# wustl-cig/FLAIR

Hardware: AMD Instinct MI355X
Metric: restored frames/sec at 256x256, 16-frame clip, 250-step DDIM (higher is better)
Workload: dtype bf16

## Files before the change

flair_amd/csrc/conv.hip:

```cpp
#include <type_traits>

#include "common.h"

namespace {

struct ConvArgs {
    const void* x[4];
    int segC[4];
    int segLd[4];
    int nseg;
    const void* w;
    const float* bias;
    const void* res0;
    const void* res1;
    int res0Ld, res1Ld;
    void* y;
    int yLd;
    int T, H, W;
    int KT, KH, KW;
    int Cout, CinTot;
    int act;
    float outScale;
    long P;
    int nPixTiles, nCoTiles;
    int tFast;
    unsigned segBytes[4];
    unsigned wBytes;
    float* part;
    int splitK;
    const float* fbias;
    int fbiasLd;
    int stride;
    int tapShift;
    int reflect;
    float actParam;
    int actPeriod;
    int Hin, Win;
    int esz;
};

template <typename E> struct Mma;

template <> struct Mma<bf16_t> {
    static constexpr int BKE = 32;
    static __device__ __forceinline__ int chunk(int i, int half) { return 2 * i + half; }
    static __device__ __forceinline__ void run(const uint4 (&a)[2], const uint4 (&b)[2], f32x16& acc) {
        acc = __builtin_amdgcn_mfma_f32_32x32x16_bf16(__builtin_bit_cast(bf16x8, a[0]),
                                                      __builtin_bit_cast(bf16x8, b[0]), acc, 0, 0, 0);
        acc = __builtin_amdgcn_mfma_f32_32x32x16_bf16(__builtin_bit_cast(bf16x8, a[1]),
                                                      __builtin_bit_cast(bf16x8, b[1]), acc, 0, 0, 0);
    }
    static __device__ __forceinline__ void run1(const uint4& a, const uint4& b, f32x16& acc) {
        acc = __builtin_amdgcn_mfma_f32_32x32x16_bf16(__builtin_bit_cast(bf16x8, a), __builtin_bit_cast(bf16x8, b),
                                                      acc, 0, 0, 0);
    }
    static constexpr int MFMA_PER_HALF = 1;
};

template <> struct Mma<float> {
    static constexpr int BKE = 16;
    static __device__ __forceinline__ int chunk(int i, int half) { return 2 * half + i; }
    static __device__ __forceinline__ void run(const uint4 (&a)[2], const uint4 (&b)[2], f32x16& acc) {
        const float* af = reinterpret_cast<const float*>(a);
        const float* bf = reinterpret_cast<const float*>(b);
#pragma unroll
        for (int s = 0; s < 8; ++s)
            acc = __builtin_amdgcn_mfma_f32_32x32x2f32(af[s], bf[s], acc, 0, 0, 0);
    }
    static __device__ __forceinline__ void run1(const uint4& a, const uint4& b, f32x16& acc) {
        const float* af = reinterpret_cast<const float*>(&a);
        const float* bf = reinterpret_cast<const float*>(&b);
#pragma unroll
        for (int s = 0; s < 4; ++s)
            acc = __builtin_amdgcn_mfma_f32_32x32x2f32(af[s], bf[s], acc, 0, 0, 0);
    }
    static constexpr int MFMA_PER_HALF = 4;
};

__device__ __forceinline__ int lds_off(int row, int chunk) {
    return row * 64 + ((chunk ^ ((row >> 2) & 3)) << 4);
}

__device__ __forceinline__ int staged_row(int id) {
    const int g = id >> 3;
    return (g >> 2) * 8 + (g & 3) + 4 * ((id >> 2) & 1);
}

template <typename E>
__device__ __forceinline__ void store_quad(const ConvArgs& a, long p, int co, float v0, float v1, float v2, float v3) {
    if (co >= a.Cout) return;
    float v[4] = {v0, v1, v2, v3};
    if (a.bias) {
        const float4 b = *reinterpret_cast<const float4*>(a.bias + co);
// ... 133 lines not shown
        }
    }
}

template <typename E, int TH, int RPW, int PF>
__global__ __launch_bounds__(64 * TH / RPW, (2 * 64 * TH / RPW + 255) / 256)
void conv3x3_halo_kernel(ConvArgs a) {
    prefetch_kernargs<sizeof(ConvArgs)>();
    constexpr int BKE = Mma<E>::BKE;
    constexpr int VEC = ET<E>::VEC;
    constexpr int NT = 64 * TH / RPW;
    constexpr int HW_ = 34;
    constexpr int PITCH = 80;
    constexpr int HALO_ROWS = (TH + 2) * HW_;
    constexpr int HALO_PIECES = (HALO_ROWS + 7) / 8 * 8 * 4;
    constexpr int W_PIECES = 64 * 9 * 4;
    constexpr int HI = (HALO_PIECES + NT - 1) / NT;
    constexpr int WI = (W_PIECES + NT - 1) / NT;
    constexpr int HALO_BYTES = (TH + 2) * HW_ * PITCH;
    extern __shared__ __attribute__((aligned(16))) char smem[];
    char* sh = smem;
    char* sw = smem + HALO_BYTES;

    const int tid = threadIdx.x, lane = tid & 63, wave = tid >> 6;
    const int lr = lane & 31, lh = lane >> 5;
    const int bid = xcd_remap(blockIdx.x, gridDim.x);
    const int coTile = bid % a.nCoTiles;
    int rest = bid / a.nCoTiles;
    const int tilesW = a.W / 32, tilesH = (a.H + TH - 1) / TH;
    const int tw = rest % tilesW;
    rest /= tilesW;
    const int th = rest % tilesH;
    const int t = rest / tilesH;
    const int h0 = th * TH, w0 = tw * 32, co0 = coTile * 64;
    const int taps = a.KT * 9;
    const int pt = a.KT / 2;

    uint4 hreg[PF][HI], wreg[PF][WI];
    int dt = -pt, seg = 0, cb = 0, segOff = 0;
    auto dt_valid = [&](int d) { return (unsigned)(t + d) < (unsigned)a.T; };
    while (dt <= pt && !dt_valid(dt)) ++dt;

    constexpr unsigned ESZ = sizeof(E);
    int hpix[HI];
    unsigned hq[HI], woff[WI];
#pragma unroll
    for (int i = 0; i < HI; ++i) {
        const int id = i * NT + tid;
        const int pix = staged_row(id);
        const int r = pix / HW_, c = pix % HW_;
        const int hh = h0 + r - 1, ww = w0 + c - 1;
        const bool ok = pix < HALO_ROWS && (unsigned)hh < (unsigned)a.H && (unsigned)ww < (unsigned)a.W;
        hpix[i] = ok ? hh * a.W + ww : -1;
        hq[i] = (id & 3) * VEC * ESZ;
    }
    const __amdgpu_buffer_rsrc_t wrs = make_rsrc(a.w, a.wBytes);
#pragma unroll
    for (int i = 0; i < WI; ++i) {
        const int id = i * NT + tid;
        const int row = staged_row(id);
        const int co = row / 9, tap9 = row % 9;
        const bool ok = id < W_PIECES && co0 + co < a.Cout;
        woff[i] = ok ? (unsigned)(((co0 + co) * taps + tap9) * a.CinTot + (id & 3) * VEC) * ESZ : FLAIR_OOB;
    }

    auto issue = [&](uint4 (&hr)[HI], uint4 (&wr)[WI]) {
        const unsigned ld = (unsigned)a.segLd[seg] * ESZ;
        const char* frame = reinterpret_cast<const char*>(a.x[seg]) + (size_t)(t + dt) * a.H * a.W * ld;
        const __amdgpu_buffer_rsrc_t xr = make_rsrc(frame, a.segBytes[seg]);
        const unsigned cofs = (unsigned)(cb * BKE) * ESZ;
#pragma unroll
        for (int i = 0; i < HI; ++i) {
            const unsigned off = hpix[i] >= 0 ? (unsigned)hpix[i] * ld + cofs + hq[i] : FLAIR_OOB;
            hr[i] = buf_load16(xr, off);
        }
        const unsigned kofs = (unsigned)((dt + pt) * 9 * a.CinTot + segOff + cb * BKE) * ESZ;
#pragma unroll
        for (int i = 0; i < WI; ++i) wr[i] = buf_load16(wrs, woff[i] == FLAIR_OOB ? FLAIR_OOB : woff[i] + kofs);
    };
    auto advance = [&]() {
        ++cb;
        if (cb * BKE >= a.segC[seg]) {
            cb = 0;
            segOff += a.segC[seg];
            if (++seg >= a.nseg) {
                seg = 0;
                segOff = 0;
                ++dt;
                while (dt <= pt && !dt_valid(dt)) ++dt;
            }
        }
    };
    auto write_lds = [&](const uint4 (&hr)[HI], const uint4 (&wr)[WI]) {
#pragma unroll
        for (int i = 0; i < HI; ++i) {
            const int id = i * NT + tid;
            const int row = staged_row(id);
            if (row < HALO_ROWS) *reinterpret_cast<uint4*>(sh + row * PITCH + (id & 3) * 16) = hr[i];
        }
#pragma unroll
        for (int i = 0; i < WI; ++i) {
            const int id = i * NT + tid;
            if (id < W_PIECES) *reinterpret_cast<uint4*>(sw + staged_row(id) * PITCH + (id & 3) * 16) = wr[i];
        }
    };
    int nValidDt = 0;
    for (int d = -pt; d <= pt; ++d) nValidDt += dt_valid(d) ? 1 : 0;
    const int nch = nValidDt * (a.CinTot / BKE);

    f32x16 acc[RPW][2];
#pragma unroll
    for (int j = 0; j < RPW; ++j)
#pragma unroll
        for (int i = 0; i < 2; ++i)
#pragma unroll
            for (int r = 0; r < 16; ++r) acc[j][i][r] = 0.f;

    auto compute = [&]() {
        const char* hb = sh + ((wave * RPW * HW_) + lr) * PITCH;
        const char* wb0 = sw + (lr * 9) * PITCH;
        const char* wb1 = sw + ((lr + 32) * 9) * PITCH;
        uint4 fa0[2][2], fa1[2][2], fb[2][RPW][2];
        auto load_tap = [&](int set, int tap9) {
            const int kh = tap9 / 3, kw = tap9 % 3;
            fa0[set][0] = *reinterpret_cast<const uint4*>(wb0 + tap9 * PITCH + 16 * Mma<E>::chunk(0, lh));
            fa0[set][1] = *reinterpret_cast<const uint4*>(wb0 + tap9 * PITCH + 16 * Mma<E>::chunk(1, lh));
            fa1[set][0] = *reinterpret_cast<const uint4*>(wb1 + tap9 * PITCH + 16 * Mma<E>::chunk(0, lh));
            fa1[set][1] = *reinterpret_cast<const uint4*>(wb1 + tap9 * PITCH + 16 * Mma<E>::chunk(1, lh));
#pragma unroll
            for (int j = 0; j < RPW; ++j) {
                const char* hp = hb + ((j + kh) * HW_ + kw) * PITCH;
                fb[set][j][0] = *reinterpret_cast<const uint4*>(hp + 16 * Mma<E>::chunk(0, lh));
                fb[set][j][1] = *reinterpret_cast<const uint4*>(hp + 16 * Mma<E>::chunk(1, lh));
            }
        };
        load_tap(0, 0);
        __builtin_amdgcn_sched_group_barrier(0x100, 4 + 2 * RPW, 0);
#pragma unroll
        for (int tap9 = 0; tap9 < 9; ++tap9) {
            const int set = tap9 & 1;
            if (tap9 < 8) load_tap(set ^ 1, tap9 + 1);
#pragma unroll
            for (int j = 0; j < RPW; ++j) {
                Mma<E>::run(fa0[set], fb[set][j], acc[j][0]);
                Mma<E>::run(fa1[set], fb[set][j], acc[j][1]);
            }
            if (tap9 < 8) __builtin_amdgcn_sched_group_barrier(0x100, 4 + 2 * RPW, 0);
            __builtin_amdgcn_sched_group_barrier(0x8, (sizeof(E) == 2 ? 4 : 16) * RPW, 0);
        }
    };

    int issued = 0;
#pragma unroll
    for (int s_ = 0; s_ < PF; ++s_)
        if (issued < nch) {
            issue(hreg[s_], wreg[s_]);
            advance();
            ++issued;
        }
    write_lds(hreg[0], wreg[0]);
    __syncthreads();
    for (int k = 0; k < nch; k += PF) {
#pragma unroll
        for (int par = 0; par < PF; ++par) {
            const int kk = k + par;
            if (kk < nch) {
                if (issued < nch) {
                    issue(hreg[par], wreg[par]);
                    advance();
                    ++issued;
                }
                compute();
                if (kk + 1 < nch) {
                    __syncthreads();
                    write_lds(hreg[(par + 1) % PF], wreg[(par + 1) % PF]);
                    __syncthreads();
                }
            }
        }
    }

    if ((a.Cout & 7) == 0) {
        constexpr int VEC = ET<E>::VEC;
        constexpr int CHUNKS = 64 / VEC;
        __syncthreads();
#pragma unroll
        for (int j = 0; j < RPW; ++j) {
            char* tile = smem + (wave * RPW + j) * 32 * (64 * 4 + 16);
#pragma unroll
            for (int i = 0; i < 2; ++i)
#pragma unroll
// ... 84 lines not shown
}

template <typename E, int TH, int RPW, int CF>
__global__ __launch_bounds__(256 * TH / RPW / CF, (256 * TH / RPW / CF) / 256) void conv3x3_halo_ks_kernel(ConvArgs a) {
    static_assert(RPW == 1 && CF == 2, "one image row and both 32-cout fragments per wave");
    prefetch_kernargs<sizeof(ConvArgs)>();
    constexpr int NRG = TH / RPW;
    constexpr int NCG = 2 / CF;
    constexpr int NW = 2 * NRG * NCG, NT = 64 * NW;
    constexpr int BKE = Mma<E>::BKE;
    constexpr int VEC = ET<E>::VEC;
    constexpr unsigned ESZ = sizeof(E);
    constexpr int HW_ = 34, PITCH = 80;
    constexpr int HALO_ROWS = (TH + 2) * HW_;
    constexpr int HALO_PIECES = (HALO_ROWS + 7) / 8 * 8 * 4;
    constexpr int W_PIECES = 64 * 9 * 4;
    constexpr int HI = (HALO_PIECES + NT - 1) / NT;
    constexpr int WI = (W_PIECES + NT - 1) / NT;
    constexpr int HALO_BYTES = (TH + 2) * HW_ * PITCH;
    constexpr int STAGE_BYTES = HALO_BYTES + 64 * 9 * PITCH;
    extern __shared__ __attribute__((aligned(16))) char smem[];

    const int tid = threadIdx.x, lane = tid & 63, wave = tid >> 6;
    const int lr = lane & 31, lh = lane >> 5;
    const int rp = wave % NRG, kh2 = (wave / NRG) & 1, cg = wave / (2 * NRG);
    const int bid = xcd_remap(blockIdx.x, gridDim.x);
    const int coTile = bid % a.nCoTiles;
    int rest = bid / a.nCoTiles;
    const int tilesW = a.W / 32, tilesH = (a.H + TH - 1) / TH;
    const int tw = rest % tilesW;
    rest /= tilesW;
    const int th = rest % tilesH;
    const int t = rest / tilesH;
    const int h0 = th * TH, w0 = tw * 32, co0 = coTile * 64;
    const int taps = a.KT * 9;
    const int pt = a.KT / 2;

    float biasv[VEC];
    {
        const int bco = co0 + (lane % (64 / VEC)) * VEC;
#pragma unroll
        for (int e = 0; e < VEC; ++e) biasv[e] = (a.bias && bco < a.Cout) ? a.bias[bco + e] : 0.f;
    }
    uint4 hreg[HI], wreg[WI];
    int dt = -pt, seg = 0, cb = 0, segOff = 0;
    auto dt_valid = [&](int d) { return (unsigned)(t + d) < (unsigned)a.T; };
    while (dt <= pt && !dt_valid(dt)) ++dt;

    int hpix[HI];
    unsigned hq[HI], woff[WI];
#pragma unroll
    for (int i = 0; i < HI; ++i) {
        const int id = i * NT + tid;
        const int pix = staged_row(id);
        const int r = pix / HW_, c = pix % HW_;
        const int hh = h0 + r - 1, ww = w0 + c - 1;
        const bool ok = pix < HALO_ROWS && (unsigned)hh < (unsigned)a.H && (unsigned)ww < (unsigned)a.W;
        hpix[i] = ok ? hh * a.W + ww : -1;
        hq[i] = (id & 3) * VEC * ESZ;
    }
    const __amdgpu_buffer_rsrc_t wrs = make_rsrc(a.w, a.wBytes);
#pragma unroll
    for (int i = 0; i < WI; ++i) {
        const int id = i * NT + tid;
        const int row = staged_row(id);
        const int co = row / 9, tap9 = row % 9;
        const bool ok = id < W_PIECES && co0 + co < a.Cout;
        woff[i] = ok ? (unsigned)(((co0 + co) * taps + tap9) * a.CinTot + (id & 3) * VEC) * ESZ : FLAIR_OOB;
    }
    auto issue = [&]() {
        const unsigned ld = (unsigned)a.segLd[seg] * ESZ;
        const char* frame = reinterpret_cast<const char*>(a.x[seg]) + (size_t)(t + dt) * a.H * a.W * ld;
        const __amdgpu_buffer_rsrc_t xr = make_rsrc(frame, a.segBytes[seg]);
        const unsigned cofs = (unsigned)(cb * BKE) * ESZ;
#pragma unroll
        for (int i = 0; i < HI; ++i)
            hreg[i] = buf_load16(xr, hpix[i] >= 0 ? (unsigned)hpix[i] * ld + cofs + hq[i] : FLAIR_OOB);
        const unsigned kofs = (unsigned)((dt + pt) * 9 * a.CinTot + segOff + cb * BKE) * ESZ;
#pragma unroll
        for (int i = 0; i < WI; ++i) wreg[i] = buf_load16(wrs, woff[i] == FLAIR_OOB ? FLAIR_OOB : woff[i] + kofs);
        ++cb;
        if (cb * BKE >= a.segC[seg]) {
            cb = 0;
            segOff += a.segC[seg];
            if (++seg >= a.nseg) {
                seg = 0;
                segOff = 0;
                ++dt;
                while (dt <= pt && !dt_valid(dt)) ++dt;
            }
        }
    };
    auto write_lds = [&](int stage) {
        char* sh = smem + stage * STAGE_BYTES;
        char* sw = sh + HALO_BYTES;
#pragma unroll
        for (int i = 0; i < HI; ++i) {
            const int id = i * NT + tid;
            const int row = staged_row(id);
            if (row < HALO_ROWS) *reinterpret_cast<uint4*>(sh + row * PITCH + (id & 3) * 16) = hreg[i];
        }
#pragma unroll
        for (int i = 0; i < WI; ++i) {
            const int id = i * NT + tid;
            if (id < W_PIECES) *reinterpret_cast<uint4*>(sw + staged_row(id) * PITCH + (id & 3) * 16) = wreg[i];
        }
    };
    int nValidDt = 0;
    for (int d = -pt; d <= pt; ++d) nValidDt += dt_valid(d) ? 1 : 0;
    const int nch = nValidDt * (a.CinTot / BKE);

    f32x16 acc[RPW][CF];
#pragma unroll
    for (int j = 0; j < RPW; ++j)
#pragma unroll
        for (int i = 0; i < CF; ++i)
#pragma unroll
            for (int r = 0; r < 16; ++r) acc[j][i][r] = 0.f;

    const int ck = 16 * Mma<E>::chunk(kh2, lh);
    auto compute = [&](int stage) {
        const char* sh = smem + stage * STAGE_BYTES;
        const char* hb = sh + ((RPW * rp * HW_) + lr) * PITCH + ck;
        const char* wb0 = sh + HALO_BYTES + ((cg * CF * 32 + lr) * 9) * PITCH + ck;
        uint4 fa[2][CF], fb[2][RPW];
        auto load_tap = [&](int set, int tap9) {
            const int kh = tap9 / 3, kw = tap9 % 3;
#pragma unroll
            for (int i = 0; i < CF; ++i)
                fa[set][i] = *reinterpret_cast<const uint4*>(wb0 + (i * 32 * 9 + tap9) * PITCH);
#pragma unroll
            for (int j = 0; j < RPW; ++j)
                fb[set][j] = *reinterpret_cast<const uint4*>(hb + ((kh + j) * HW_ + kw) * PITCH);
        };
        load_tap(0, 0);
        __builtin_amdgcn_sched_group_barrier(0x100, CF + RPW, 0);
#pragma unroll
        for (int tap9 = 0; tap9 < 9; ++tap9) {
            const int set = tap9 & 1;
            if (tap9 < 8) load_tap(set ^ 1, tap9 + 1);
#pragma unroll
            for (int j = 0; j < RPW; ++j)
#pragma unroll
                for (int i = 0; i < CF; ++i) Mma<E>::run1(fa[set][i], fb[set][j], acc[j][i]);
            if (tap9 < 8) __builtin_amdgcn_sched_group_barrier(0x100, CF + RPW, 0);
            __builtin_amdgcn_sched_group_barrier(0x8, CF * RPW * Mma<E>::MFMA_PER_HALF, 0);
        }
    };

    issue();
    write_lds(0);
    if (nch > 1) issue();
    __syncthreads();
    for (int k = 0; k < nch; ++k) {
        compute(k & 1);
        if (k + 1 < nch) {
            write_lds((k + 1) & 1);
            if (k + 2 < nch) issue();
            __syncthreads();
        }
    }

    constexpr int FPITCH = 64 * 4 + 16;
    constexpr int CHUNKS = 64 / VEC;
    constexpr int PARTS = NW / TH;
    constexpr int NIT = 32 * CHUNKS / 64 / PARTS;
    const int orow = wave % TH, part = wave / TH;
    const int h = h0 + orow;
    const long prow = ((long)t * a.H + h) * a.W + w0;
    const int ech = lane % CHUNKS;
    const int eco = co0 + ech * VEC;
    const bool eok = h < a.H && eco < a.Cout;
    uint4 r0v[NIT], r1v[NIT];
#pragma unroll
    for (int k = 0; k < NIT; ++k) {
        const int px = ((k * PARTS + part) * 64 + lane) / CHUNKS;
        const long p = prow + px;
        r0v[k] = r1v[k] = make_uint4(0u, 0u, 0u, 0u);
        if (eok && a.res0) r0v[k] = *reinterpret_cast<const uint4*>(reinterpret_cast<const E*>(a.res0) + p * a.res0Ld + eco);
        if (eok && a.res1) r1v[k] = *reinterpret_cast<const uint4*>(reinterpret_cast<const E*>(a.res1) + p * a.res1Ld + eco);
    }
    __syncthreads();
#pragma unroll
    for (int pass = 0; pass < 2; ++pass) {
        if (kh2 == pass) {
#pragma unroll
            for (int j = 0; j < RPW; ++j) {
                char* tile = smem + (RPW * rp + j) * 32 * FPITCH + lr * FPITCH;
#pragma unroll
                for (int i = 0; i < CF; ++i)
#pragma unroll
                    for (int g = 0; g < 4; ++g) {
                        float4* dst = reinterpret_cast<float4*>(tile + ((cg * CF + i) * 32 + 8 * g + 4 * lh) * 4);
// ... 20 lines not shown
        float v[VEC];
        const float* src = reinterpret_cast<const float*>(tile + px * FPITCH) + ech * VEC;
#pragma unroll
        for (int e = 0; e < VEC; e += 4) {
            const float4 q = *reinterpret_cast<const float4*>(src + e);
            v[e] = q.x; v[e + 1] = q.y; v[e + 2] = q.z; v[e + 3] = q.w;
        }
#pragma unroll
        for (int e = 0; e < VEC; ++e) v[e] += biasv[e];
        if (a.fbias) {
            const float* fb = a.fbias + (long)t * a.fbiasLd + eco;
#pragma unroll
            for (int e = 0; e < VEC; ++e) v[e] += fb[e];
        }
        if (leaky) {
#pragma unroll
            for (int e = 0; e < VEC; ++e) v[e] = fmaxf(v[e], v[e] * slope);
        } else if (a.act == FLAIR_ACT_DCN_OFFSETS) {
            dcn_offset_act<VEC>(v, eco, a.actParam, a.actPeriod);
        } else if (a.act == FLAIR_ACT_SILU) {
#pragma unroll
            for (int e = 0; e < VEC; ++e) v[e] = silu_f(v[e]);
        } else {
#pragma unroll
            for (int e = 0; e < VEC; ++e) v[e] = apply_act(v[e], a.act);
        }
        if (a.res0) {
            float r[VEC];
            Vec16<E>::load(reinterpret_cast<const E*>(&r0v[k]), r);
#pragma unroll
            for (int e = 0; e < VEC; ++e) v[e] += r[e];
        }
        if (a.res1) {
            float r[VEC];
            Vec16<E>::load(reinterpret_cast<const E*>(&r1v[k]), r);
#pragma unroll
            for (int e = 0; e < VEC; ++e) v[e] += r[e];
        }
#pragma unroll
        for (int e = 0; e < VEC; ++e) v[e] *= a.outScale;
        Vec16<E>::store(reinterpret_cast<E*>(a.y) + p * a.yLd + eco, v);
    }
}

template <typename E, int TH, int RPW, int CF>
int launch_halo_ks(const ConvArgs& a0, hipStream_t s) {
    ConvArgs a = a0;
    a.nCoTiles = cdiv(a.Cout, 64);
    const int grid = a.T * cdiv(a.H, TH) * (a.W / 32) * a.nCoTiles;
    const size_t lds = 2 * ((size_t)(TH + 2) * 34 * 80 + 64 * 9 * 80);
    static LdsAttrOnce attr;
    {
        const hipError_t e = flair_max_lds_once(attr, reinterpret_cast<const void*>(&conv3x3_halo_ks_kernel<E, TH, RPW, CF>));
        FLAIR_CHECK(e == hipSuccess, "flair_conv_nhwc: hipFuncSetAttribute: %s", hipGetErrorString(e));
    }
    hipLaunchKernelGGL((conv3x3_halo_ks_kernel<E, TH, RPW, CF>), dim3(grid), dim3(256 * TH / RPW / CF), lds, s, a);
    FLAIR_LAUNCH_CHECK();
    return FLAIR_OK;
}

struct DmaTile {
    int t, h0, w0, co0;
};

template <int NW, int RPW, int NSTAGE>
__device__ __forceinline__ void conv3x3_dma_body(const ConvArgs& a, int nTiles, int tilesPerXcd) {
    using E = bf16_t;
    static_assert((RPW == 1 || RPW == 2) && NSTAGE == 2, "the clip-level and one-tile forms (two stages)");
    constexpr int KSTEPS = 2;
    constexpr int TH = NW * RPW, HWP = 34;
    constexpr int HALO_ROWS = (TH + 2) * HWP;
    constexpr int HALO_INSTR = (HALO_ROWS + 15) / 16;
    constexpr int W_INSTR = 64 * 9 / 16;
    constexpr int HALO_BYTES = HALO_INSTR * 1024;
    constexpr int STAGE_BYTES = HALO_BYTES + W_INSTR * 1024;
    constexpr int NSLOT = (HALO_INSTR + W_INSTR + NW - 1) / NW;
    constexpr int BIAS_OFF = NSTAGE * STAGE_BYTES + NW * 1024;
    extern __shared__ __attribute__((aligned(16))) char smem[];

    const int tid = threadIdx.x, lane = tid & 63;
    const int wave = __builtin_amdgcn_readfirstlane(tid >> 6);
    const int lr = lane & 31, lh = lane >> 5;
    const int taps = a.KT * 9, pt = a.KT / 2;
    const int chunksPerTap = a.CinTot / 32;
    const int H = a.H, W = a.W, T = a.T;

    const int xcd = blockIdx.x & 7, slot = blockIdx.x >> 3, slotsPerXcd = gridDim.x >> 3;
    const int tilesW = W / 32, tilesH = H / TH, nCoTiles = a.nCoTiles;
    auto tile_at = [&](int i, DmaTile& tl) -> bool {
        const int inXcd = slot + i * slotsPerXcd;
        const int id = xcd * tilesPerXcd + inXcd;
        if (inXcd >= tilesPerXcd || id >= nTiles) return false;
        int rest = id;
        tl.co0 = (rest % nCoTiles) * 64;
        rest /= nCoTiles;
        if (a.tFast) {
            tl.t = rest % T;
            rest /= T;
            tl.w0 = (rest % tilesW) * 32;
            tl.h0 = (rest / tilesW) * TH;
            return true;
        }
        tl.w0 = (rest % tilesW) * 32;
        rest /= tilesW;
        tl.h0 = (rest % tilesH) * TH;
        tl.t = rest / tilesH;
        return true;
    };

    const int lrow = lane >> 2, lchunk = lane & 3;
    unsigned slotv[NSLOT], hchunk[NSLOT];
#pragma unroll
    for (int i = 0; i < NSLOT; ++i) {
        const int id = wave * NSLOT + i;
        const int c = (id * 16 + lrow) % HWP;
        hchunk[i] = (unsigned)((lchunk ^ ((c >> 2) & 3)) << 4);
    }
    auto setup_tile = [&](const DmaTile& tl) {
#pragma unroll
        for (int i = 0; i < NSLOT; ++i) {
            const int id = wave * NSLOT + i;
            const int R = id * 16 + lrow;
            const int hr = R / HWP, c = R - hr * HWP;
            const int hh = tl.h0 - 1 + hr, ww = tl.w0 - 1 + c;
            const bool okh = R < HALO_ROWS && (unsigned)hh < (unsigned)H && (unsigned)ww < (unsigned)W;
            const unsigned hv = okh ? (unsigned)(hh * W + ww) : 0xffffffffu;
            const int row = R - HALO_INSTR * 16;
            const int tap9 = row >> 6, co = row & 63;
            const bool okw = row >= 0 && row < 576 && tl.co0 + co < a.Cout;
            const unsigned wv = okw ? (unsigned)(((tl.co0 + co) * taps + tap9) * a.CinTot) * 2u + ((lchunk ^ ((co >> 2) & 3)) << 4) : FLAIR_OOB;
            slotv[i] = id >= HALO_INSTR ? wv : hv;
        }
    };

    const u32x4_t wdesc = make_desc(a.w, a.wBytes);
    struct Walk {
        int dt, seg, cb, segOff, j;
    };
    auto dt_at = [&](int t, int j) { return a.tFast ? (j + a.KT * T - t) % a.KT - pt : j - pt; };
    auto walk_first = [&](int t, Walk& wk) {
        wk.j = 0; wk.seg = 0; wk.cb = 0; wk.segOff = 0;
        while (wk.j < a.KT && (unsigned)(t + dt_at(t, wk.j)) >= (unsigned)T) ++wk.j;
        wk.dt = dt_at(t, wk.j);
    };
    auto walk_next = [&](int t, Walk& wk) {
        ++wk.cb;
        if (wk.cb * 32 >= a.segC[wk.seg]) {
            wk.cb = 0;
            wk.segOff += a.segC[wk.seg];
            if (++wk.seg >= a.nseg) {
                wk.seg = 0;
                wk.segOff = 0;
                ++wk.j;
                while (wk.j < a.KT && (unsigned)(t + dt_at(t, wk.j)) >= (unsigned)T) ++wk.j;
                wk.dt = dt_at(t, wk.j);
            }
        }
    };
    auto chunks_of = [&](int t) {
        int n = 0;
        for (int d = -pt; d <= pt; ++d) n += (unsigned)(t + d) < (unsigned)T ? 1 : 0;
        return n * chunksPerTap;
    };
    auto issue = [&](const DmaTile& tl, const Walk& wk, int stage) {
        const unsigned ld = (unsigned)a.segLd[wk.seg] * 2u;
        const char* frame = reinterpret_cast<const char*>(a.x[wk.seg]) + (size_t)(tl.t + wk.dt) * H * W * ld;
        const u32x4_t xdesc = make_desc(frame, a.segBytes[wk.seg]);
        const unsigned cofs = (unsigned)(wk.cb * 64);
        const unsigned kofs = (unsigned)((wk.dt + pt) * 9 * a.CinTot + wk.segOff + wk.cb * 32) * 2u;
        const unsigned sbase = (unsigned)(stage * STAGE_BYTES + wave * NSLOT * 1024);
#pragma unroll
        for (int i = 0; i < NSLOT; ++i) {
            const bool isw = wave * NSLOT + i >= HALO_INSTR;
            const unsigned sv = slotv[i];
            const unsigned offh = sv == 0xffffffffu ? FLAIR_OOB : sv * ld + cofs + hchunk[i];
            const unsigned offw = sv == FLAIR_OOB ? FLAIR_OOB : sv + kofs;
            u32x4_t d;
            d.x = isw ? wdesc.x : xdesc.x;
            d.y = isw ? wdesc.y : xdesc.y;
            d.z = isw ? wdesc.z : xdesc.z;
            d.w = 0x00020000u;
            const bool idle = wave * NSLOT + i >= HALO_INSTR + W_INSTR;
            dma16(d, isw ? offw : offh, idle ? (unsigned)(NSTAGE * STAGE_BYTES + ((wave * NSLOT + i - HALO_INSTR - W_INSTR) % NW) * 1024) : sbase + i * 1024);
        }
    };

    unsigned aoff[KSTEPS], boff[3][KSTEPS];
#pragma unroll
    for (int s_ = 0; s_ < KSTEPS; ++s_) {
        aoff[s_] = (unsigned)(HALO_BYTES + lr * 64 + (((2 * s_ + lh) ^ ((lr >> 2) & 3)) << 4));
#pragma unroll
        for (int kw = 0; kw < 3; ++kw)
            boff[kw][s_] = (unsigned)((RPW * wave * HWP + kw + lr) * 64 + (((2 * s_ + lh) ^ (((kw + lr) >> 2) & 3)) << 4));
    }

    f32x16 acc[RPW][2];
    auto zero_acc = [&]() {
#pragma unroll
        for (int j = 0; j < RPW; ++j)
#pragma unroll
            for (int i = 0; i < 2; ++i)
#pragma unroll
                for (int r = 0; r < 16; ++r) acc[j][i][r] = 0.f;
    };
    auto compute = [&](int stage) {
        const char* sb = smem + stage * STAGE_BYTES;
        uint4 fb[2][RPW + 2][KSTEPS];
        uint4 fa[2][2][KSTEPS];
        auto load_b = [&](int set, int kw) {
#pragma unroll
            for (int h = 0; h < RPW + 2; ++h)
#pragma unroll
                for (int s_ = 0; s_ < KSTEPS; ++s_)
                    fb[set][h][s_] = *reinterpret_cast<const uint4*>(sb + h * (HWP * 64) + boff[kw][s_]);
        };
        auto load_a = [&](int set, int kh, int kw) {
#pragma unroll
            for (int cf = 0; cf < 2; ++cf)
#pragma unroll
                for (int s_ = 0; s_ < KSTEPS; ++s_)
                    fa[set][cf][s_] = *reinterpret_cast<const uint4*>(sb + (kh * 3 + kw) * 4096 + cf * 2048 + aoff[s_]);
        };
        load_b(0, 0);
        load_a(0, 0, 0);
        __builtin_amdgcn_sched_group_barrier(0x100, KSTEPS * (RPW + 2) + 2 * KSTEPS, 0);
#pragma unroll
        for (int step = 0; step < 9; ++step) {
            const int kq = step / 3, kh = step % 3;
            const int nkq = (step + 1) / 3, nkh = (step + 1) % 3;
            if (step < 8) {
                if (nkh == 0) load_b(nkq & 1, nkq);
                load_a((step + 1) & 1, nkh, nkq);
            }
#pragma unroll
            for (int j = 0; j < RPW; ++j)
#pragma unroll
                for (int cf = 0; cf < 2; ++cf) Mma<E>::run(fa[step & 1][cf], fb[kq & 1][j + kh], acc[j][cf]);
            if (step < 8) {
                if (nkh == 0) __builtin_amdgcn_sched_group_barrier(0x100, KSTEPS * (RPW + 2) + 2 * KSTEPS, 0);
// ... 209 lines not shown
            if (more) {
                walk_first(nxt.t, wk);
                setup_tile(nxt);
                remIssue = chunks_of(nxt.t);
                bias_request(nxt);
            }
        }
        if (more) {
            issue(nxt, wk, stage ^ 1);
            walk_next(nxt.t, wk);
            --remIssue;
        }
        compute(stage);
        if (biasPending) bias_commit(iNxt);
        bool storesInFlight = false;
        if (--remCompute == 0) {
            epilogue(cur, iCur);
            storesInFlight = RPW >= 2 ? !a.res1 : cur.co0 + 64 <= a.Cout && !res0any;
            ++iCur;
            if (!tile_at(iCur, cur)) break;
            remCompute = chunks_of(cur.t);
            zero_acc();
        }
        if (storesInFlight) {
            asm volatile("s_waitcnt vmcnt(%0)" ::"n"(4 * RPW) : "memory");
        } else {
            asm volatile("s_waitcnt vmcnt(0)" ::: "memory");
        }
        __syncthreads();
        stage ^= 1;
    }
}

template <int NW, int RPW, int NSTAGE>
__global__ __launch_bounds__(64 * NW, (NW + 3) / 4) void conv3x3_dma_kernel(ConvArgs a, int nTiles, int tilesPerXcd) {
    prefetch_kernargs<sizeof(ConvArgs) + 8>();
    conv3x3_dma_body<NW, RPW, NSTAGE>(a, nTiles, tilesPerXcd);
}

template <int NW, int RPW, int NSTAGE>
int launch_dma(const ConvArgs& a0, hipStream_t s) {
    constexpr int TH = NW * RPW;
    ConvArgs a = a0;
    a.nCoTiles = cdiv(a.Cout, 64);
    a.tFast = a.KT == 3 && a.T > 1;
    const int nTiles = a.T * (a.H / TH) * (a.W / 32) * a.nCoTiles;
    const int nCu = flair_cu_count();
    int grid = nTiles < nCu ? (nTiles + 7) / 8 * 8 : nCu / 8 * 8;
    if (grid < 8) grid = 8;
    const int tilesPerXcd = (nTiles + 7) / 8;
    constexpr int HALO_INSTR = ((TH + 2) * 34 + 15) / 16;
    const size_t lds = NSTAGE * (size_t)(HALO_INSTR + 36) * 1024 + NW * 1024 + 512;
    static LdsAttrOnce attr;
    {
        const hipError_t e = flair_max_lds_once(attr, reinterpret_cast<const void*>(&conv3x3_dma_kernel<NW, RPW, NSTAGE>));
        FLAIR_CHECK(e == hipSuccess, "flair_conv_nhwc: hipFuncSetAttribute: %s", hipGetErrorString(e));
    }
    hipLaunchKernelGGL((conv3x3_dma_kernel<NW, RPW, NSTAGE>), dim3(grid), dim3(64 * NW), lds, s, a, nTiles, tilesPerXcd);

    FLAIR_LAUNCH_CHECK();
    return FLAIR_OK;
}


template <bool HALO3>
__global__ __launch_bounds__(512, 2) void conv_frame_kernel(ConvArgs a) {
    static_assert(HALO3, "halo ring of three, weight ring of two");
    prefetch_kernargs<sizeof(ConvArgs)>();
    using E = bf16_t;
    constexpr int NW = 8, HWP = 34;
    constexpr int HINSTR = 22, HIMG = HINSTR * 1024, WINSTR = 36, SLOT = WINSTR * 1024;
    constexpr int HR = 3, WR = 2;
    constexpr int RING = HR * HIMG, BIAS = RING + WR * SLOT;
    constexpr int NH = (HINSTR + NW - 1) / NW, NWS = (WINSTR + NW - 1) / NW;
    extern __shared__ __attribute__((aligned(16))) char smem[];
    const int tid = threadIdx.x, lane = tid & 63;
    const int wave = __builtin_amdgcn_readfirstlane(tid >> 6);
    const int lr = lane & 31, lh = lane >> 5;
    const int lrow = lane >> 2, lchunk = lane & 3;
    const int tilesW = a.W / 32, perFrame = tilesW * (a.H / 8);
    const int bid = xcd_remap(blockIdx.x, gridDim.x);
    const int t = bid / perFrame, tile = bid - t * perFrame;
    const int h0 = (tile / tilesW) * 8, w0 = (tile % tilesW) * 32;
    const int nS = a.CinTot / 32;

    const u32x4_t wdesc = make_desc(a.w, a.wBytes);
    const u32x4_t bdesc = make_desc(a.bias, a.bias ? (unsigned)a.Cout * 4u : 0u);
    dma16(bdesc, (unsigned)(lane * 16), (unsigned)BIAS);
    unsigned hpix[NH], hpiece[NH];
#pragma unroll
    for (int i = 0; i < NH; ++i) {
        const int k = (wave * NH + i) % HINSTR;
        const int R = k * 16 + lrow;
        const int hr = R / HWP, c = R - hr * HWP;
        const int hh = h0 - 1 + hr, ww = w0 - 1 + c;
        const bool ok = R < 10 * HWP && (unsigned)hh < (unsigned)a.H && (unsigned)ww < (unsigned)a.W;
        hpix[i] = ok ? (unsigned)(hh * a.W + ww) : 0xffffffffu;
        hpiece[i] = (unsigned)((lchunk ^ ((c >> 2) & 3)) << 4);
    }
    unsigned wlane[NWS];
#pragma unroll
    for (int i = 0; i < NWS; ++i) {
        const int id = (wave * NWS + i) % WINSTR;
        const int row = id * 16 + lrow, tap9 = row >> 6, co = row & 63;
        wlane[i] = co < a.Cout ? (unsigned)((co * 9 + tap9) * a.CinTot) * 2u + (unsigned)((lchunk ^ ((co >> 2) & 3)) << 4) : FLAIR_OOB;
    }
    int hseg = 0, hcb = 0;
    auto issue_halo = [&](int slot) {
        const unsigned ld = (unsigned)a.segLd[hseg] * 2u;
        const u32x4_t xdesc = make_desc(reinterpret_cast<const char*>(a.x[hseg]) + (size_t)t * a.H * a.W * ld, a.segBytes[hseg]);
        const unsigned cofs = (unsigned)(hcb * 64);
#pragma unroll
        for (int i = 0; i < NH; ++i) {
            const int k = (wave * NH + i) % HINSTR;
            dma16(xdesc, hpix[i] == 0xffffffffu ? FLAIR_OOB : hpix[i] * ld + cofs + hpiece[i], (unsigned)(slot * HIMG + k * 1024));
        }
        if (++hcb * 32 >= a.segC[hseg]) {
            hcb = 0;
            ++hseg;
        }
    };
    auto issue_w = [&](int s_) {
#pragma unroll
        for (int i = 0; i < NWS; ++i) {
            const int id = (wave * NWS + i) % WINSTR;
            dma16(wdesc, wlane[i] == FLAIR_OOB ? FLAIR_OOB : wlane[i] + (unsigned)(s_ * 64), (unsigned)(RING + (s_ % WR) * SLOT + id * 1024));
        }
    };
    issue_halo(0);
    issue_w(0);
    if (nS > 1) {
        issue_halo(1);
        issue_w(1);
    }
    if (nS > 2) issue_halo(2);

    unsigned aoff[2], boff[3][2];
#pragma unroll
    for (int ks = 0; ks < 2; ++ks) {
        aoff[ks] = (unsigned)(lr * 64 + (((2 * ks + lh) ^ ((lr >> 2) & 3)) << 4));
#pragma unroll
        for (int kw = 0; kw < 3; ++kw)
            boff[kw][ks] = (unsigned)((wave * HWP + kw + lr) * 64 + (((2 * ks + lh) ^ (((kw + lr) >> 2) & 3)) << 4));
    }
    f32x16 acc[2];
    auto compute = [&](int wslot, int hslot) {
        const char* wb = smem + RING + wslot * SLOT;
        const char* xb = smem + hslot * HIMG;
        uint4 fb[2][3][2], fa[2][2][2];
        auto load_b = [&](int set, int kw) {
#pragma unroll
            for (int h = 0; h < 3; ++h)
#pragma unroll
                for (int ks = 0; ks < 2; ++ks) fb[set][h][ks] = *reinterpret_cast<const uint4*>(xb + h * (HWP * 64) + boff[kw][ks]);
        };
        auto load_a = [&](int set, int kh, int kw) {
#pragma unroll
            for (int cf = 0; cf < 2; ++cf)
#pragma unroll
                for (int ks = 0; ks < 2; ++ks) fa[set][cf][ks] = *reinterpret_cast<const uint4*>(wb + (kh * 3 + kw) * 4096 + cf * 2048 + aoff[ks]);
        };
        load_b(0, 0);
        load_a(0, 0, 0);
#pragma unroll
        for (int step = 0; step < 9; ++step) {
            const int kq = step / 3, kh = step % 3;
            const int nkq = (step + 1) / 3, nkh = (step + 1) % 3;
            if (step < 8) {
                if (nkh == 0) load_b(nkq & 1, nkq);
                load_a((step + 1) & 1, nkh, nkq);
            }
#pragma unroll
            for (int cf = 0; cf < 2; ++cf)
#pragma unroll
                for (int ks = 0; ks < 2; ++ks)
                    acc[cf] = __builtin_amdgcn_mfma_f32_32x32x16_bf16(__builtin_bit_cast(bf16x8, fa[step & 1][cf][ks]), __builtin_bit_cast(bf16x8, fb[kq & 1][kh][ks]), acc[cf], 0, 0, 0);
        }
    };

    const long prow = ((long)t * a.H + h0 + wave) * a.W + w0;
    const unsigned yLdB = (unsigned)a.yLd * 2u, r0LdB = (unsigned)a.res0Ld * 2u, r1LdB = (unsigned)a.res1Ld * 2u;
    const __amdgpu_buffer_rsrc_t yd = make_rsrc(reinterpret_cast<char*>(a.y) + prow * a.yLd * 2, (unsigned)a.W * yLdB);
    const __amdgpu_buffer_rsrc_t r0d = make_rsrc(a.res0 ? reinterpret_cast<const char*>(a.res0) + prow * a.res0Ld * 2 : nullptr, a.res0 ? (unsigned)a.W * r0LdB : 0u);
    const __amdgpu_buffer_rsrc_t r1d = make_rsrc(a.res1 ? reinterpret_cast<const char*>(a.res1) + prow * a.res1Ld * 2 : nullptr, a.res1 ? (unsigned)a.W * r1LdB : 0u);
    uint4 r0v[4], r1v[4];
#pragma unroll
    for (int g = 0; g < 4; ++g) r0v[g] = r1v[g] = make_uint4(0u, 0u, 0u, 0u);

    for (int s_ = 0; s_ < nS; ++s_) {
        if (s_ + 1 >= nS) asm volatile("s_waitcnt vmcnt(0)" ::: "memory");
        else if (s_ == 0 && nS > 2) asm volatile("s_waitcnt vmcnt(%0)" ::"n"(2 * NH + NWS) : "memory");
        else if (s_ == 0) asm volatile("s_waitcnt vmcnt(%0)" ::"n"(NH + NWS) : "memory");
        else asm volatile("s_waitcnt vmcnt(%0)" ::"n"(NH) : "memory");
        __builtin_amdgcn_s_barrier();
        if (s_ == 0) {
            const float* sb = reinterpret_cast<const float*>(smem + BIAS);
#pragma unroll
            for (int cf = 0; cf < 2; ++cf)
#pragma unroll
                for (int g = 0; g < 4; ++g) {
                    const float4 bq = *reinterpret_cast<const float4*>(sb + cf * 32 + 8 * g + 4 * lh);
                    acc[cf][4 * g] = bq.x; acc[cf][4 * g + 1] = bq.y; acc[cf][4 * g + 2] = bq.z; acc[cf][4 * g + 3] = bq.w;
                }
        }
        if (s_ >= 1 && s_ + 1 < nS) issue_w(s_ + 1);
        if (s_ >= 1 && s_ + 2 < nS) issue_halo((s_ + 2) % 3);
        if (s_ + 1 == nS) {
            if (a.res0) {
#pragma unroll
// ... 27 lines not shown
            Vec16<E>::load(reinterpret_cast<const E*>(&r0v[g]), r);
#pragma unroll
            for (int e = 0; e < 8; ++e) v[e] += r[e];
            Vec16<E>::load(reinterpret_cast<const E*>(&r1v[g]), r);
#pragma unroll
            for (int e = 0; e < 8; ++e) v[e] = (v[e] + r[e]) * scale;
            alignas(16) E out[8];
            Vec16<E>::store(out, v);
            const uint4 ov = *reinterpret_cast<const uint4*>(out);
            const unsigned yo = 16 * g + 8 * lh < a.Cout ? (unsigned)lr * yLdB + (unsigned)(32 * g + 16 * lh) : FLAIR_OOB;
            __builtin_amdgcn_raw_buffer_store_b128(u32x4_t{ov.x, ov.y, ov.z, ov.w}, yd, (int)yo, 0, 0);
        }
}

static bool frame_kernel_ok(const ConvArgs& a) {
    if (a.esz != 2 || a.KT != 1 || a.KH != 3 || a.KW != 3 || a.stride != 1 || a.fbias || a.Cout > 64 || a.Cout % 8 || a.W % 32 || a.H % 8) return false;
    if (!(a.act == FLAIR_ACT_NONE || a.act == FLAIR_ACT_RELU || a.act == FLAIR_ACT_LRELU01 || a.act == FLAIR_ACT_LRELU02)) return false;
    if (a.tapShift || a.reflect || a.CinTot % 32 || a.CinTot < 32) return false;
    for (int i = 0; i < a.nseg; ++i)
        if (a.segC[i] % 32) return false;
    return true;
}

static int launch_frame(const ConvArgs& a, hipStream_t s) {
    constexpr size_t lds = (3 * 22 + 2 * 36) * 1024 + 1024;
    static LdsAttrOnce attr;
    const hipError_t e = flair_max_lds_once(attr, reinterpret_cast<const void*>(&conv_frame_kernel<true>));
    FLAIR_CHECK(e == hipSuccess, "flair_conv_nhwc: hipFuncSetAttribute: %s", hipGetErrorString(e));
    hipLaunchKernelGGL(conv_frame_kernel<true>, dim3(a.T * (a.H / 8) * (a.W / 32)), dim3(512), lds, s, a);
    FLAIR_LAUNCH_CHECK();
    return FLAIR_OK;
}

template <typename E, int TC, int TP, int WC, int WP, int PD, int KWID>
__global__ __launch_bounds__(256) void conv_igemm_kernel(ConvArgs a) {
    prefetch_kernargs<sizeof(ConvArgs)>();
    constexpr int BKE = Mma<E>::BKE * KWID;
    constexpr int ROWB = 64 * KWID;
    constexpr int CPR = 4 * KWID;
    constexpr int RPP = 256 / CPR;
    constexpr int VEC = ET<E>::VEC;
    constexpr int FC = TC / WC / 32;
    constexpr int FP = TP / WP / 32;
    constexpr int XR = TP / RPP;
    constexpr int WR = TC / RPP;
    static_assert(WC * WP == 4 && FC >= 1 && FP >= 1 && XR >= 1 && WR >= 1, "tile");

    extern __shared__ __attribute__((aligned(16))) char smem[];
    constexpr int BUF = (TC + TP) * ROWB;
    auto loff = [](int row, int chunk) { return KWID == 1 ? lds_off(row, chunk) : row * 128 + ((chunk ^ ((row >> 1) & 7)) << 4); };

    const int tid = threadIdx.x;
    const int lane = tid & 63, wave = __builtin_amdgcn_readfirstlane(tid >> 6);
    const int wc = wave / WP, wp = wave % WP;

    const int bid = xcd_remap(blockIdx.x, gridDim.x);
    const int coTile = bid % a.nCoTiles;
    const int pixTile = bid / a.nCoTiles;
    const long p0 = (long)pixTile * TP;
    const int co0 = coTile * TC;

    const int chunk = tid % CPR;
    const int srow = tid / CPR;
    int xt[XR], xh[XR], xw[XR];
    bool xvalid[XR];
#pragma unroll
    for (int i = 0; i < XR; ++i) {
        long p = p0 + srow + RPP * i;
        xvalid[i] = p < a.P;
        if (!xvalid[i]) p = 0;
        int w_ = (int)(p % a.W);
        long q = p / a.W;
        xw[i] = w_;
        xh[i] = (int)(q % a.H);
        xt[i] = (int)(q / a.H);
    }
    const int taps = a.KT * a.KH * a.KW;
    const int pt = a.KT / 2, ph = a.KH / 2, pw = a.KW / 2;
    const int tFirst = (int)(p0 / ((long)a.H * a.W));
    const int tileFrames = (int)((TP + (long)a.H * a.W - 1) / ((long)a.H * a.W)) + 1;

    uint4 xreg[PD][XR], wreg[PD][WR];

    const int nkAll = taps * (a.CinTot / BKE);
    const int ks0 = (int)((long)blockIdx.y * nkAll / a.splitK);
    const int ks1 = (int)((long)(blockIdx.y + 1) * nkAll / a.splitK);
    int tap = ks0 / (a.CinTot / BKE), seg = 0, cb = ks0 % (a.CinTot / BKE), segOff = 0;
    while (cb * BKE >= a.segC[seg]) {
        cb -= a.segC[seg] / BKE;
        segOff += a.segC[seg];
        ++seg;
    }
    int dw = tap % a.KW - pw, dh = (tap / a.KW) % a.KH - ph, dt = tap / (a.KW * a.KH) - pt;

    const __amdgpu_buffer_rsrc_t wrs = make_rsrc(a.w, a.wBytes);
    constexpr unsigned ESZ = sizeof(E);
    auto issue_loads = [&](int set) {
        const int ld = a.segLd[seg];
        int fb = tFirst + dt;
        fb = fb < 0 ? 0 : (fb >= a.T ? a.T - 1 : fb);
        int nfr = a.T - fb;
        if (nfr > tileFrames) nfr = tileFrames;
        const size_t frameBytes = (size_t)a.Hin * a.Win * ld * ESZ;
        const __amdgpu_buffer_rsrc_t xr =
            make_rsrc(reinterpret_cast<const char*>(a.x[seg]) + fb * frameBytes, (unsigned)(nfr * frameBytes));
        const int coff = cb * BKE + chunk * VEC;
#pragma unroll
        for (int i = 0; i < XR; ++i) {
            const int t2 = xt[i] + dt;
            int h2 = xh[i] * a.stride + dh + a.tapShift, w2 = xw[i] * a.stride + dw + a.tapShift;
            if (a.reflect) {
                h2 = h2 < 0 ? -h2 : (h2 >= a.Hin ? 2 * a.Hin - 2 - h2 : h2);
                w2 = w2 < 0 ? -w2 : (w2 >= a.Win ? 2 * a.Win - 2 - w2 : w2);
            }
            const bool ok = xvalid[i] && (unsigned)t2 < (unsigned)a.T && (unsigned)h2 < (unsigned)a.Hin &&
                            (unsigned)w2 < (unsigned)a.Win;
            const unsigned off = ok ? (unsigned)((((t2 - fb) * a.Hin + h2) * a.Win + w2) * ld + coff) * ESZ : FLAIR_OOB;
            xreg[set][i] = buf_load16(xr, off);
        }
        const unsigned kofs = (unsigned)(tap * a.CinTot + segOff + coff) * ESZ;
#pragma unroll
        for (int j = 0; j < WR; ++j) {
            const int n = co0 + srow + RPP * j;
            wreg[set][j] = buf_load16(wrs, n < a.Cout ? (unsigned)(n * taps * a.CinTot) * ESZ + kofs : FLAIR_OOB);
        }
    };
    auto advance = [&]() {
        ++cb;
        if (cb * BKE >= a.segC[seg]) {
            cb = 0;
            segOff += a.segC[seg];
            ++seg;
            if (seg >= a.nseg) {
                seg = 0;
                segOff = 0;
                ++tap;
                ++dw;
                if (dw > pw) {
                    dw = -pw;
                    ++dh;
                    if (dh > ph) {
                        dh = -ph;
                        ++dt;
                    }
                }
            }
        }
    };
    auto write_lds = [&](int buf, int set) {
        char* base = smem + buf * BUF;
#pragma unroll
        for (int j = 0; j < WR; ++j)
            *reinterpret_cast<uint4*>(base + loff(srow + RPP * j, chunk)) = wreg[set][j];
#pragma unroll
        for (int i = 0; i < XR; ++i)
            *reinterpret_cast<uint4*>(base + TC * ROWB + loff(srow + RPP * i, chunk)) = xreg[set][i];
    };

    f32x16 acc[FC][FP];
#pragma unroll
    for (int i = 0; i < FC; ++i)
#pragma unroll
        for (int j = 0; j < FP; ++j)
#pragma unroll
            for (int r = 0; r < 16; ++r) acc[i][j][r] = 0.f;

    const int nk = ks1 - ks0;
    const int lr = lane & 31, lh = lane >> 5;

#pragma unroll
    for (int u = 0; u < PD; ++u)
        if (u < nk) {
            issue_loads(u);
            advance();
        }
    write_lds(0, 0);
    __syncthreads();

    for (int ks = 0; ks < nk; ks += PD) {
#pragma unroll
        for (int u = 0; u < PD; ++u) {
            const int k = ks + u;
            if (k >= nk) break;
            const int cur = k & 1;
            if (k + PD < nk) {
                issue_loads(u);
                advance();
            }
            const char* wb = smem + cur * BUF;
            const char* xb = wb + TC * ROWB;
#pragma unroll
            for (int sp = 0; sp < KWID; ++sp) {
                uint4 af[FC][2], bfr[FP][2];
#pragma unroll
                for (int i = 0; i < FC; ++i) {
                    const int row = wc * (TC / WC) + i * 32 + lr;
                    af[i][0] = *reinterpret_cast<const uint4*>(wb + loff(row, 4 * sp + Mma<E>::chunk(0, lh)));
                    af[i][1] = *reinterpret_cast<const uint4*>(wb + loff(row, 4 * sp + Mma<E>::chunk(1, lh)));
                }
#pragma unroll
                for (int j = 0; j < FP; ++j) {
                    const int row = wp * (TP / WP) + j * 32 + lr;
                    bfr[j][0] = *reinterpret_cast<const uint4*>(xb + loff(row, 4 * sp + Mma<E>::chunk(0, lh)));
                    bfr[j][1] = *reinterpret_cast<const uint4*>(xb + loff(row, 4 * sp + Mma<E>::chunk(1, lh)));
                }
#pragma unroll
                for (int i = 0; i < FC; ++i)
#pragma unroll
                    for (int j = 0; j < FP; ++j) Mma<E>::run(af[i], bfr[j], acc[i][j]);
            }
            if (k + 1 < nk) write_lds(cur ^ 1, (u + 1) % PD);
            __syncthreads();
        }
    }

    if (a.splitK > 1) {
#pragma unroll
        for (int j = 0; j < FP; ++j) {
            const long p = p0 + wp * (TP / WP) + j * 32 + lr;
            if (p >= a.P) continue;
#pragma unroll
            for (int i = 0; i < FC; ++i)
#pragma unroll
                for (int g = 0; g < 4; ++g) {
                    const int co = co0 + wc * (TC / WC) + i * 32 + 8 * g + 4 * lh;
                    if (co < a.Cout)
                        *reinterpret_cast<float4*>(a.part + ((long)blockIdx.y * a.P + p) * a.Cout + co) =
                            make_float4(acc[i][j][4 * g], acc[i][j][4 * g + 1], acc[i][j][4 * g + 2],
                                        acc[i][j][4 * g + 3]);
                }
        }
        return;
    }
    if ((a.Cout & 7) == 0 && ((uintptr_t)a.y & 15) == 0 && (a.yLd * (int)sizeof(E)) % 16 == 0 &&
        (!a.res0 || (((uintptr_t)a.res0 & 15) == 0 && (a.res0Ld * (int)sizeof(E)) % 16 == 0)) &&
        (!a.res1 || (((uintptr_t)a.res1 & 15) == 0 && (a.res1Ld * (int)sizeof(E)) % 16 == 0))) {
        auto run = [&](auto actTag) {
            igemm_epilogue<E, decltype(actTag)::value, FC, FP>(a, acc, p0 + wp * (TP / WP), co0 + wc * (TC / WC), lr, lh);
        };
        if (a.act == FLAIR_ACT_DCN_OFFSETS) run(std::integral_constant<int, 1>{});
        else if (a.act == FLAIR_ACT_SILU) run(std::integral_constant<int, 2>{});
        else if (a.act == FLAIR_ACT_GELU) run(std::integral_constant<int, 3>{});
        else run(std::integral_constant<int, 0>{});
        return;
    }
#pragma unroll
    for (int j = 0; j < FP; ++j) {
        const long p = p0 + wp * (TP / WP) + j * 32 + lr;
        if (p >= a.P) continue;
#pragma unroll
        for (int i = 0; i < FC; ++i)
#pragma unroll
            for (int g = 0; g < 4; ++g)
                store_quad<E>(a, p, co0 + wc * (TC / WC) + i * 32 + 8 * g + 4 * lh, acc[i][j][4 * g],
                              acc[i][j][4 * g + 1], acc[i][j][4 * g + 2], acc[i][j][4 * g + 3]);
    }
}

template <typename E>
__global__ void conv_splitk_reduce_kernel(ConvArgs a) {
    const unsigned cq = (unsigned)(a.Cout / 4);
    const unsigned quads = (unsigned)a.P * cq;
    const size_t slice = (size_t)a.P * a.Cout;
    for (unsigned i = blockIdx.x * blockDim.x + threadIdx.x; i < quads; i += gridDim.x * blockDim.x) {
        const unsigned p = i / cq;
        const int co = (int)(i - p * cq) * 4;
        const float* src = a.part + (size_t)p * a.Cout + co;
        float4 s = make_float4(0.f, 0.f, 0.f, 0.f);
        int k = 0;
        for (; k + 4 <= a.splitK; k += 4) {
            float4 v[4];
#pragma unroll
            for (int u = 0; u < 4; ++u) v[u] = *reinterpret_cast<const float4*>(src + (size_t)(k + u) * slice);
#pragma unroll
            for (int u = 0; u < 4; ++u) {
                s.x += v[u].x; s.y += v[u].y; s.z += v[u].z; s.w += v[u].w;
            }
        }
        for (; k < a.splitK; ++k) {
            const float4 v = *reinterpret_cast<const float4*>(src + (size_t)k * slice);
            s.x += v.x; s.y += v.y; s.z += v.z; s.w += v.w;
        }
        store_quad<E>(a, p, co, s.x, s.y, s.z, s.w);
    }
}

template <typename E, int TC, int TP, int WC, int WP, int PD, int KWID>
int launch_pd(const ConvArgs& a0, hipStream_t s) {
    ConvArgs a = a0;
    a.nPixTiles = cdiv(a.P, TP);
    a.nCoTiles = cdiv(a.Cout, TC);
    const int grid = a.nPixTiles * a.nCoTiles;
    const size_t lds = 2 * (TC + TP) * 64 * KWID;
    hipLaunchKernelGGL((conv_igemm_kernel<E, TC, TP, WC, WP, PD, KWID>), dim3(grid, a.splitK), dim3(256), lds, s, a);
    FLAIR_LAUNCH_CHECK();
    if (a.splitK > 1) {
        long g = (a.P * (a.Cout / 4) + 255) / 256;
        if (g > 2048) g = 2048;
        hipLaunchKernelGGL(conv_splitk_reduce_kernel<E>, dim3((int)g), dim3(256), 0, s, a);
        FLAIR_LAUNCH_CHECK();
    }
    return FLAIR_OK;
}

template <typename E, int TC, int TP, int WC, int WP>
int launch(const ConvArgs& a, hipStream_t s) {
    if constexpr (sizeof(E) == 2) {
        bool ok = true;
        for (int i = 0; i < a.nseg; ++i) ok = ok && a.segC[i] % 64 == 0;
        if (ok) return launch_pd<E, TC, TP, WC, WP, 2, 2>(a, s);
    }
    return launch_pd<E, TC, TP, WC, WP, 4, 1>(a, s);
}

int choose_split(const ConvArgs& a, int variant) {
    if (variant > 2) return 1;
    const int maxBlocks = variant == 0 ? 512 : 1024, maxSplit = 16;
    const int tc = variant == 0 ? 128 : 64, tp = variant == 2 ? 64 : 128;
    const int bke = 64 / (a.wBytes && a.CinTot ? (int)(a.wBytes / ((unsigned long long)a.Cout * a.KT * a.KH * a.KW * a.CinTot)) : 2);
    const long nk = (long)a.KT * a.KH * a.KW * (a.CinTot / bke);
    const long tiles = (long)cdiv(a.P, tp) * cdiv(a.Cout, tc);
    if (tiles >= 384 || nk < 32) return 1;
    long s = maxBlocks / tiles;
    if (s > maxSplit) s = maxSplit;
    if (s > nk / 8) s = nk / 8;
    return s < 1 ? 1 : (int)s;
}

int choose_variant(const ConvArgs& a) {
    if (!a.reflect && a.stride == 1 && a.KH == 3 && a.KW == 3 && a.W % 32 == 0 && a.H >= 2) {
        const long per = (long)a.T * (a.W / 32) * cdiv(a.Cout, 64);
        const bool ks = a.Cout % 8 == 0;
        if (a.esz == 2 && ks && a.act != FLAIR_ACT_GELU && a.H % 16 == 0 && per * cdiv(a.H, 8) > 256 && per * (a.H / 16) >= 192) return 8;
        const bool dmaOk = a.esz == 2 && ks && a.act != FLAIR_ACT_GELU;
        if (per * cdiv(a.H, 8) >= 256) return ks && per * cdiv(a.H, 8) <= 256 ? (dmaOk && a.H % 8 == 0 ? 9 : 6) : 3;
        if (per * cdiv(a.H, 4) >= 256) return ks && per * cdiv(a.H, 4) <= 256 ? 7 : 4;
        return 5;
    }
    const long tiles128 = (long)cdiv(a.P, 128) * cdiv(a.Cout, 128);
    if (a.Cout > 64 && tiles128 >= 512) return 0;
    if (a.Cout >= 128 && a.P >= 1024 && tiles128 <= 64 && (long)a.KT * a.KH * a.KW * a.CinTot >= 2304) return 0;
    const long tiles64x128 = (long)cdiv(a.P, 128) * cdiv(a.Cout, 64);
    if (tiles64x128 >= 512) return 1;
    return 2;
}

template <typename E>
int dispatch(const ConvArgs& a0, hipStream_t s) {
    ConvArgs a = a0;
    const int variant = choose_variant(a);
    a.splitK = a.part ? choose_split(a, variant) : 1;
    switch (variant) {
        case 0: return launch<E, 128, 128, 2, 2>(a, s);
        case 1: return launch<E, 64, 128, 1, 4>(a, s);
        case 2: return launch<E, 64, 64, 2, 2>(a, s);
        case 3: return launch_halo<E, 8, 1, 1>(a, s);
        case 4: return launch_halo<E, 4, 1, 1>(a, s);
        case 6: return launch_halo_ks<E, 8, 1, 2>(a, s);
        case 7: return launch_halo_ks<E, 4, 1, 2>(a, s);
        case 8: return launch_dma<8, 2, 2>(a, s);
        case 9:
            if (frame_kernel_ok(a)) return launch_frame(a, s);
            return launch_dma<8, 1, 2>(a, s);
        default: return launch_halo<E, 2, 1, 1>(a, s);
    }
}

}

extern "C" int flair_conv_variant(const flair_conv_params* p);

static void fill_geometry(ConvArgs& a, const flair_conv_params* p) {
    a.stride = p->stride > 1 ? p->stride : 1;
    a.Hin = p->H; a.Win = p->W;
    a.T = p->T; a.KT = p->KT; a.KH = p->KH; a.KW = p->KW; a.Cout = p->Cout;
    a.reflect = p->reflect_pad ? 1 : 0;
    a.act = p->act;
    a.H = (p->H + a.stride - 1) / a.stride;
    a.W = (p->W + a.stride - 1) / a.stride;
    a.P = (long)p->T * a.H * a.W;
    a.CinTot = 0;
    for (int i = 0; i < p->nseg && i < 4; ++i) a.CinTot += p->seg_c[i];
    const int esz = p->dtype == FLAIR_BF16 ? 2 : 4;
    a.esz = esz;
    a.wBytes = (unsigned)((unsigned long long)p->Cout * p->KT * p->KH * p->KW * a.CinTot * esz);
}

extern "C" size_t flair_conv_workspace_bytes(const flair_conv_params* p) {
    if (!p) return 0;
    ConvArgs a{};
    fill_geometry(a, p);
    const int split = choose_split(a, choose_variant(a));
    return split > 1 ? (size_t)split * a.P * a.Cout * sizeof(float) : 0;
}

extern "C" int flair_conv_nhwc(const flair_conv_params* p, const void* const* x, const void* w,
                               const float* bias, const float* frame_bias, const void* res0, const void* res1,
                               void* y, void* workspace, size_t workspace_bytes, hipStream_t stream) {
    FLAIR_CHECK(p && x && w && y, "flair_conv_nhwc: null argument");
    FLAIR_CHECK(p->dtype == FLAIR_F32 || p->dtype == FLAIR_BF16, "flair_conv_nhwc: bad dtype %d", p->dtype);
    FLAIR_CHECK(p->nseg >= 1 && p->nseg <= 4, "flair_conv_nhwc: nseg %d not in 1..4", p->nseg);
    FLAIR_CHECK(p->T > 0 && p->H > 0 && p->W > 0 && p->Cout > 0, "flair_conv_nhwc: empty shape");
    FLAIR_CHECK((p->KT & 1) && (p->KH & 1) && (p->KW & 1), "flair_conv_nhwc: kernel taps must be odd");
    FLAIR_CHECK(p->Cout % 4 == 0, "flair_conv_nhwc: Cout %d must be a multiple of 4", p->Cout);
    const int bke = p->dtype == FLAIR_BF16 ? 32 : 16;
    const int esz = p->dtype == FLAIR_BF16 ? 2 : 4;
    ConvArgs a{};
    a.CinTot = 0;
    for (int i = 0; i < p->nseg; ++i) {
        FLAIR_CHECK(x[i], "flair_conv_nhwc: segment %d is null", i);
        FLAIR_CHECK(p->seg_c[i] > 0 && p->seg_c[i] % bke == 0,
                    "flair_conv_nhwc: segment %d has %d channels; must be a multiple of %d", i, p->seg_c[i], bke);
        FLAIR_CHECK(p->seg_ld[i] >= p->seg_c[i] && (p->seg_ld[i] * esz) % 16 == 0 &&
                        ((uintptr_t)x[i]) % 16 == 0,
                    "flair_conv_nhwc: segment %d stride/alignment", i);
        a.x[i] = x[i];
        a.segC[i] = p->seg_c[i];
        a.segLd[i] = p->seg_ld[i];
        a.CinTot += p->seg_c[i];
        const unsigned long long bytes = (unsigned long long)p->H * p->W * p->seg_ld[i] * esz;
        FLAIR_CHECK(bytes < 0x40000000ull, "flair_conv_nhwc: one frame of segment %d spans %llu bytes (limit 1 GiB)",
                    i, bytes);
        a.segBytes[i] = (unsigned)bytes;
    }
    {
        const unsigned long long wb = (unsigned long long)p->Cout * p->KT * p->KH * p->KW * a.CinTot * esz;
        FLAIR_CHECK(wb < 0x80000000ull, "flair_conv_nhwc: weights span %llu bytes (limit 2 GiB)", wb);
        a.wBytes = (unsigned)wb;
    }
    const int gran = (p->dtype == FLAIR_BF16 && p->Cout % 8 != 0) ? 8 : 16;
    FLAIR_CHECK(p->y_ld >= p->Cout && (p->y_ld * esz) % gran == 0 && ((uintptr_t)y) % 16 == 0,
                "flair_conv_nhwc: output stride/alignment (y_ld = %d: >= Cout = %d, a multiple of %d bytes; y 16-byte aligned)",
                p->y_ld, p->Cout, gran);
    FLAIR_CHECK(!res0 || (p->res_ld[0] >= p->Cout && (p->res_ld[0] * esz) % gran == 0 && ((uintptr_t)res0) % gran == 0),
                "flair_conv_nhwc: res0 stride/alignment (res_ld = %d: >= Cout = %d; stride and pointer multiples of %d bytes)",
                p->res_ld[0], p->Cout, gran);
    FLAIR_CHECK(!res1 || (p->res_ld[1] >= p->Cout && (p->res_ld[1] * esz) % gran == 0 && ((uintptr_t)res1) % gran == 0),
                "flair_conv_nhwc: res1 stride/alignment (res_ld = %d: >= Cout = %d; stride and pointer multiples of %d bytes)",
                p->res_ld[1], p->Cout, gran);
    FLAIR_CHECK(((uintptr_t)w) % 16 == 0, "flair_conv_nhwc: weight alignment");
    FLAIR_CHECK(!bias || ((uintptr_t)bias) % 16 == 0, "flair_conv_nhwc: bias alignment");
    a.nseg = p->nseg;
    a.w = w;
    a.bias = bias;
    a.fbias = frame_bias;
    a.fbiasLd = p->frame_bias_ld;
    FLAIR_CHECK(!frame_bias || p->frame_bias_ld >= p->Cout, "flair_conv_nhwc: frame_bias_ld");
    {
        const unsigned long long hw = (unsigned long long)p->H * p->W * esz;
        FLAIR_CHECK(hw * p->y_ld < 0x40000000ull && (!res0 || hw * p->res_ld[0] < 0x40000000ull) && (!res1 || hw * p->res_ld[1] < 0x40000000ull),
                    "flair_conv_nhwc: one frame of the output / a residual spans more than 1 GiB");
    }
    a.res0 = res0;
    a.res1 = res1;
    a.res0Ld = p->res_ld[0];
    a.res1Ld = p->res_ld[1];
    a.y = y;
    a.yLd = p->y_ld;
    a.act = p->act;
    a.actParam = p->act_param;
    a.actPeriod = p->act_period;
    FLAIR_CHECK(p->act != FLAIR_ACT_DCN_OFFSETS || (p->act_period > 0 && p->act_period % 24 == 0),
                "flair_conv_nhwc: FLAIR_ACT_DCN_OFFSETS needs act_period = 3 * deform_groups (multiple of 24), got %d",
                p->act_period);
    a.outScale = p->out_scale;
    {
        ConvArgs g{};
        fill_geometry(g, p);
        a.stride = g.stride; a.Hin = g.Hin; a.Win = g.Win; a.T = g.T; a.H = g.H; a.W = g.W; a.P = g.P;
        a.KT = g.KT; a.KH = g.KH; a.KW = g.KW; a.Cout = g.Cout; a.esz = g.esz;
    }
    FLAIR_CHECK(a.stride == 1 || a.stride == 2, "flair_conv_nhwc: stride %d unsupported", p->stride);
    FLAIR_CHECK(!p->asym_pad || (a.stride == 2 && a.KH == a.KW && a.KT == 1 && p->H % 2 == 0 && p->W % 2 == 0),
                "flair_conv_nhwc: asym_pad needs a square 2-D stride-2 kernel on even frames");
    a.tapShift = p->asym_pad ? a.KH / 2 : 0;
    FLAIR_CHECK(!p->reflect_pad || (!p->asym_pad && a.KT == 1 && p->H > a.KH / 2 && p->W > a.KW / 2),
                "flair_conv_nhwc: reflect_pad needs a 2-D kernel smaller than the frame");
    a.reflect = p->reflect_pad ? 1 : 0;
    a.part = nullptr;
    a.splitK = 1;

    if (workspace && workspace_bytes >= flair_conv_workspace_bytes(p) && flair_conv_workspace_bytes(p) > 0) {
        FLAIR_CHECK(((uintptr_t)workspace) % 16 == 0, "flair_conv_nhwc: workspace alignment");
        a.part = reinterpret_cast<float*>(workspace);
    }
    if (p->dtype == FLAIR_BF16) return dispatch<bf16_t>(a, stream);
    return dispatch<float>(a, stream);
}

extern "C" int flair_conv_variant(const flair_conv_params* p) {
    if (!p) return -1;
    ConvArgs a{};
    fill_geometry(a, p);
    return choose_variant(a);
}
```

flair_amd/csrc/dcn.hip:

```cpp


#include "common.h"

namespace {

struct DcnArgs {
    const void* x[2];
    int xLd[2];
    int Cin;
    const void* raw; int rawLd;
    const float* flow1;
    const float* flow2;
    const void* w;
    const float* bias;
    void* y; int yLd;
    int F, H, W, Cout, G;
    float maxMag;
    int activated;
    long P;
    unsigned xBytes[2], rawBytes, wBytes;
};

template <typename E> struct MmaD;
template <> struct MmaD<bf16_t> {
// ... 29 lines not shown

__device__ __forceinline__ unsigned cvt_pk_bf16(float lo, float hi) {
    unsigned r;
    asm("v_cvt_pk_bf16_f32 %0, %1, %2" : "=v"(r) : "v"(lo), "v"(hi));
    return r;
}

__device__ __forceinline__ float fast_tanh(float x) {
    const float e = __expf(2.f * x);
    return 1.f - 2.f * __builtin_amdgcn_rcpf(e + 1.f);
}

template <typename E, int NCF, int NPF, int TPP, int OFFS, bool ONEFRAME, int PFD, bool DOT2>
__global__ __launch_bounds__(32 * NPF * TPP, (PFD == 1 ? 8 : NCF >= 4 ? 32 * NPF * TPP / 256 : 4)) void dcn_kernel(DcnArgs a) {
    static_assert(DOT2 == (sizeof(E) == 2 && OFFS == 1 && ONEFRAME), "the dot2 blend exactly for the bf16 per-frame activated forms");
    static_assert(OFFS != 2 || !ONEFRAME, "raw offsets: the general (batched) form only");
    prefetch_kernargs<sizeof(DcnArgs)>();
    constexpr int NT = 32 * NPF * TPP, NW = NT / 64;

    constexpr int TP = 32 * NPF, TC = 32 * NCF, CPR = TPP;
    constexpr int VEC = ET<E>::VEC;
    constexpr unsigned ESZ = sizeof(E);
    constexpr int BKE = CPR * VEC;
    constexpr int NPAIR = NCF * NPF;
    constexpr int KSPLIT = NW > NPAIR ? NW / NPAIR : 1;
    constexpr int PAIRS = NW > NPAIR ? 1 : NPAIR / NW;
    constexpr int KSUB = CPR / 4 / KSPLIT;
    static_assert((NW > NPAIR ? NPAIR * KSPLIT == NW : PAIRS * NW == NPAIR) && KSUB >= 1 && KSUB * KSPLIT * 4 == CPR,
                  "tile shape");
    constexpr int WR = (TC * CPR + NT - 1) / NT;
    constexpr int RAWR = (TP * 3 * (int)ESZ + NT - 1) / NT;
    constexpr int BUF = (TC + TP) * CPR * 16;
    extern __shared__ __attribute__((aligned(16))) char smem[];
    const int G = a.G;
    const int slabBytes = OFFS == 2 ? (3 * G * (int)ESZ + 15) & ~15 : 3 * G * (int)ESZ;
    const int slabPieces = slabBytes / 16;
    const int rawPitch = slabBytes + 16;
    char* sraw = smem;
    char* stile = smem + 2 * TP * rawPitch;

    const int tid = threadIdx.x, lane = tid & 63, wave = tid >> 6;
    const int lr = lane & 31, lh = lane >> 5;
    const long p0 = (long)xcd_remap(blockIdx.x, gridDim.x) * TP;
    const int q = tid % TPP, srow = tid / TPP;
    long p = p0 + srow;
    const bool pvalid = p < a.P;
    if (!pvalid) p = a.P - 1;
    const int pw = (int)(p % a.W);
    const int ph = (int)((p / a.W) % a.H);
    const int pf = (int)((ONEFRAME ? p0 : p) / ((long)a.W * a.H));
    float2 fl1 = make_float2(0.f, 0.f), fl2 = make_float2(0.f, 0.f);
    if (a.flow1) fl1 = *reinterpret_cast<const float2*>(a.flow1 + p * 2);
    if (a.flow2) fl2 = *reinterpret_cast<const float2*>(a.flow2 + p * 2);

    const __amdgpu_buffer_rsrc_t rr = make_rsrc(a.raw, a.rawBytes);
    auto raw_issue = [&](int tap, uint4 (&reg)[RAWR]) {
#pragma unroll
        for (int j = 0; j < RAWR; ++j) {
            const int id = tid + j * NT;
            const int px = id / slabPieces, pc = id - px * slabPieces;
            const long pp = p0 + px;
            const unsigned within = (unsigned)(3 * tap * G) * ESZ + pc * 16;
            reg[j] = buf_load16(rr, px < TP && pp < a.P ? (unsigned)(pp * a.rawLd * ESZ) + within : FLAIR_OOB);
        }
    };
    auto raw_write = [&](int tap, const uint4 (&reg)[RAWR]) {
#pragma unroll
        for (int j = 0; j < RAWR; ++j) {
            const int id = tid + j * NT;
            const int px = id / slabPieces, pc = id - px * slabPieces;
            if (px < TP) *reinterpret_cast<uint4*>(sraw + ((tap & 1) * TP + px) * rawPitch + pc * 16) = reg[j];
        }
    };
    auto stage_raw = [&](int tap) {
        uint4 reg[RAWR];
        raw_issue(tap, reg);
        raw_write(tap, reg);
    };

    const int cpg = a.Cin / G;
    int cpgShift = 0;
    while ((1 << cpgShift) < cpg) ++cpgShift;
    const int halfC = a.Cin / 2;
    const int cbPerTap = a.Cin / BKE;
    const int nk = 9 * cbPerTap;
    const size_t fo0 = ONEFRAME ? (size_t)pf * a.H * a.W * a.xLd[0] * ESZ : 0, fo1 = ONEFRAME ? (size_t)pf * a.H * a.W * a.xLd[1] * ESZ : 0;
    const __amdgpu_buffer_rsrc_t xr0 = make_rsrc(reinterpret_cast<const char*>(a.x[0]) + fo0, a.xBytes[0]);
    const __amdgpu_buffer_rsrc_t xr1 = make_rsrc(reinterpret_cast<const char*>(a.x[1]) + fo1, a.xBytes[1]);
    const __amdgpu_buffer_rsrc_t wrs = make_rsrc(a.w, a.wBytes);
    const unsigned frameBase = (unsigned)pf * a.H * a.W;

    struct Regs {
        uint4 c[4];
        uint4 w[WR];
        float wt[4];
    } rs[PFD];

    unsigned wrow[WR];
#pragma unroll
    for (int j = 0; j < WR; ++j) {
        const int id = tid + j * NT;
        const int n = id / CPR, ch = id % CPR;
        wrow[j] = n < a.Cout && n < TC ? (unsigned)(n * 9 * a.Cin + ch * VEC) * ESZ : FLAIR_OOB;
    }
    int itap = 0, icb = 0, ikh = 0, ikw = 0;
    const int rawRow = srow * rawPitch;
    const float fH = (float)a.H, fW = (float)a.W;
    const float phm1 = (float)(ph - 1), pwm1 = (float)(pw - 1);
    auto issue = [&](Regs& r) {
        const int tap = itap, cb = icb;
        const int c = cb * BKE + q * VEC;
        const int g = c >> cpgShift;
        const E* myraw = reinterpret_cast<const E*>(sraw + (tap & 1) * TP * rawPitch + rawRow);
        const float ry = ET<E>::ld(myraw + 2 * g), rx = ET<E>::ld(myraw + 2 * g + 1);
        const float rm = ET<E>::ld(myraw + 2 * G + g);
        const bool second = cb * BKE >= halfC;
        const float2 fl = second ? fl2 : fl1;
        float sy = phm1 + (float)ikh + fl.y, sx = pwm1 + (float)ikw + fl.x, mk;
        if constexpr (OFFS == 1) {
            sy += ry;
            sx += rx;
            mk = rm;
        } else if constexpr (OFFS == 2) {
            sy += ry;
            sx += rx;
            mk = __builtin_amdgcn_rcpf(1.f + __expf(-rm));
        } else {
            sy += a.maxMag * fast_tanh(ry);
            sx += a.maxMag * fast_tanh(rx);
            mk = __builtin_amdgcn_rcpf(1.f + __expf(-rm));
        }
        const float fy = floorf(sy), fx = floorf(sx);
        const float ay = sy - fy, ax = sx - fx;
        const int y0 = (int)__builtin_amdgcn_fmed3f(fy, -2.f, fH), x0 = (int)__builtin_amdgcn_fmed3f(fx, -2.f, fW);
        const unsigned ld = (unsigned)(second ? a.xLd[1] : a.xLd[0]) * ESZ;
        const unsigned coff = (unsigned)(c - (second ? halfC : 0)) * ESZ;
        const __amdgpu_buffer_rsrc_t xr = second ? xr1 : xr0;
        const unsigned rowStep = (unsigned)a.W * ld;
        if constexpr (ONEFRAME) {
            const float wx0 = (unsigned)x0 < (unsigned)a.W ? (1.f - ax) * mk : 0.f;
            const float wx1 = (unsigned)(x0 + 1) < (unsigned)a.W ? ax * mk : 0.f;
            r.wt[0] = (1.f - ay) * wx0;
            r.wt[1] = (1.f - ay) * wx1;
            r.wt[2] = ay * wx0;
            r.wt[3] = ay * wx1;
            const unsigned o00 =
                (unsigned)mul_i24(mul_i24(y0, a.W) + x0, (int)ld) + coff;
            r.c[0] = buf_load16(xr, o00);
            r.c[1] = buf_load16(xr, o00 + ld);
            r.c[2] = buf_load16(xr, o00 + rowStep);
            r.c[3] = buf_load16(xr, o00 + rowStep + ld);
        } else {
            r.wt[0] = (1.f - ay) * (1.f - ax) * mk;
            r.wt[1] = (1.f - ay) * ax * mk;
            r.wt[2] = ay * (1.f - ax) * mk;
            r.wt[3] = ay * ax * mk;
            const unsigned o00 = (unsigned)mul_i24(
                                     (int)frameBase + mul_i24(y0, a.W) + x0, (int)ld) + coff;
            const bool yok0 = pvalid && (unsigned)y0 < (unsigned)a.H, yok1 = pvalid && (unsigned)(y0 + 1) < (unsigned)a.H;
            const bool xok0 = (unsigned)x0 < (unsigned)a.W, xok1 = (unsigned)(x0 + 1) < (unsigned)a.W;
            r.c[0] = buf_load16(xr, yok0 && xok0 ? o00 : FLAIR_OOB);
            r.c[1] = buf_load16(xr, yok0 && xok1 ? o00 + ld : FLAIR_OOB);
            r.c[2] = buf_load16(xr, yok1 && xok0 ? o00 + rowStep : FLAIR_OOB);
            r.c[3] = buf_load16(xr, yok1 && xok1 ? o00 + rowStep + ld : FLAIR_OOB);
        }
        const unsigned wk = (unsigned)(tap * a.Cin + cb * BKE) * ESZ;
#pragma unroll
// ... 35 lines not shown
            outv = make_uint4(o[0], o[1], o[2], o[3]);
        } else if constexpr (sizeof(E) == 2) {
            typedef float f32x2 __attribute__((ext_vector_type(2)));
            f32x2 lo[2] = {{0.f, 0.f}, {0.f, 0.f}}, hi[2] = {{0.f, 0.f}, {0.f, 0.f}};
#pragma unroll
            for (int i = 0; i < 4; ++i) {
                const unsigned d[4] = {r.c[i].x, r.c[i].y, r.c[i].z, r.c[i].w};
                const f32x2 w = {r.wt[i], r.wt[i]};
#pragma unroll
                for (int j = 0; j < 2; ++j) {
                    const f32x2 vl = {__uint_as_float(d[2 * j] << 16), __uint_as_float(d[2 * j + 1] << 16)};
                    const f32x2 vh = {__uint_as_float(d[2 * j] & 0xffff0000u), __uint_as_float(d[2 * j + 1] & 0xffff0000u)};
                    lo[j] = __builtin_elementwise_fma(w, vl, lo[j]);
                    hi[j] = __builtin_elementwise_fma(w, vh, hi[j]);
                }
            }
            outv = make_uint4(cvt_pk_bf16(lo[0].x, hi[0].x), cvt_pk_bf16(lo[0].y, hi[0].y), cvt_pk_bf16(lo[1].x, hi[1].x),
                              cvt_pk_bf16(lo[1].y, hi[1].y));
        } else {
            float acc[VEC];
#pragma unroll
            for (int e = 0; e < VEC; ++e) acc[e] = 0.f;
#pragma unroll
            for (int i = 0; i < 4; ++i) {
                float v[VEC];
                Vec16<E>::load(reinterpret_cast<const E*>(&r.c[i]), v);
#pragma unroll
                for (int e = 0; e < VEC; ++e) acc[e] = fmaf(r.wt[i], v[e], acc[e]);
            }
            alignas(16) E out[VEC];
            Vec16<E>::store(out, acc);
            outv = *reinterpret_cast<const uint4*>(out);
        }
        *reinterpret_cast<uint4*>(base + TC * CPR * 16 + tile_off<CPR>(srow, q)) = outv;
#pragma unroll
        for (int j = 0; j < WR; ++j) {
            const int id = tid + j * NT;
            if (id < TC * CPR) *reinterpret_cast<uint4*>(base + tile_off<CPR>(id / CPR, id % CPR)) = r.w[j];
        }
    };

    f32x16 acc[PAIRS];
#pragma unroll
    for (int i = 0; i < PAIRS; ++i)
#pragma unroll
        for (int r = 0; r < 16; ++r) acc[i][r] = 0.f;

    constexpr int LEAD = PFD + 1;
    int stageTap = 0;
    {
        uint4 r0[RAWR], r1[RAWR];
        const bool two = cbPerTap - LEAD < 0;
        raw_issue(0, r0);
        if (two) raw_issue(1, r1);
        raw_write(0, r0);
        if (two) raw_write(1, r1);
        stageTap = two ? 2 : 1;
    }
    int stageAt = stageTap * cbPerTap - LEAD;
    __syncthreads();
    auto mfma_step = [&](int buf) {
        const char* wb = stile + buf * BUF;
        const char* xb = wb + TC * CPR * 16;
#pragma unroll
        for (int i = 0; i < PAIRS; ++i) {
            const int pair = KSPLIT > 1 ? wave % NPAIR : wave * PAIRS + i;
            const int kpart = KSPLIT > 1 ? wave / NPAIR : 0;
            const int pfrag = pair % NPF, cf = pair / NPF;
#pragma unroll
            for (int kk = 0; kk < KSUB; ++kk) {
                const int ks = kpart * KSUB + kk;
                uint4 af[2], bf[2];
#pragma unroll
                for (int h = 0; h < 2; ++h) {
                    const int ch = ks * 4 + MmaD<E>::chunk(h, lh);
                    bf[h] = *reinterpret_cast<const uint4*>(xb + tile_off<CPR>(pfrag * 32 + lr, ch));
                    af[h] = *reinterpret_cast<const uint4*>(wb + tile_off<CPR>(cf * 32 + lr, ch));
                }
                MmaD<E>::run(af, bf, acc[i]);
            }
        }
    };
#pragma unroll
    for (int u = 0; u < PFD - 1; ++u)
        if (u < nk) issue(rs[u]);
    constexpr int UNR = 2 * PFD;
    for (int k = 0; k < nk; k += UNR) {
#pragma unroll
        for (int u = 0; u < UNR; ++u) {
            if (k + u < nk) {
                if (k + u + PFD - 1 < nk) issue(rs[(u + PFD - 1) % PFD]);
                blend_and_stage(rs[u % PFD], u & 1);
                __syncthreads();
                mfma_step(u & 1);
                if (k + u == stageAt && stageTap < 9) {
                    stage_raw(stageTap);
                    ++stageTap;
                    stageAt += cbPerTap;
                }
            }
        }
    }
    if constexpr (KSPLIT > 1) {
        __syncthreads();
        float* red = reinterpret_cast<float*>(stile);
        const int pair0 = wave % NPAIR, kpart0 = wave / NPAIR;
        if (kpart0 > 0) {
            float* dst = red + ((kpart0 - 1) * NPAIR + pair0) * 64 * 16 + lane * 16;
#pragma unroll
            for (int r = 0; r < 16; r += 4)
                *reinterpret_cast<float4*>(dst + r) = make_float4(acc[0][r], acc[0][r + 1], acc[0][r + 2], acc[0][r + 3]);
        }
        __syncthreads();
        if (kpart0 > 0) return;
#pragma unroll
        for (int kp = 1; kp < KSPLIT; ++kp) {
            const float* src = red + ((kp - 1) * NPAIR + pair0) * 64 * 16 + lane * 16;
#pragma unroll
            for (int r = 0; r < 16; r += 4) {
                const float4 v = *reinterpret_cast<const float4*>(src + r);
                acc[0][r] += v.x; acc[0][r + 1] += v.y; acc[0][r + 2] += v.z; acc[0][r + 3] += v.w;
            }
        }
    }
    E* y = reinterpret_cast<E*>(a.y);
    if constexpr (sizeof(E) == 2) {
        if ((a.Cout & 7) == 0 && (a.yLd & 7) == 0 && (reinterpret_cast<uintptr_t>(a.y) & 15) == 0) {
            const __amdgpu_buffer_rsrc_t bd = make_rsrc(a.bias, a.bias ? (unsigned)a.Cout * 4u : 0u);
            const __amdgpu_buffer_rsrc_t yd = make_rsrc(a.y, (unsigned)a.P * a.yLd * 2u);
#pragma unroll
            for (int i = 0; i < PAIRS; ++i) {
                const int pair = KSPLIT > 1 ? wave % NPAIR : wave * PAIRS + i;
                const int pfrag = pair % NPF, cf = pair / NPF;
                const long po = p0 + pfrag * 32 + lr;
                uint4 bq[2][2];
#pragma unroll
                for (int j = 0; j < 2; ++j) {
                    const int co = cf * 32 + 16 * j + 8 * lh;
                    bq[j][0] = buf_load16(bd, co < a.Cout ? 4u * co : FLAIR_OOB);
                    bq[j][1] = buf_load16(bd, co < a.Cout ? 4u * co + 16u : FLAIR_OOB);
                }
#pragma unroll
                for (int j = 0; j < 2; ++j) {
                    const int co = cf * 32 + 16 * j + 8 * lh;
                    float v[8];
#pragma unroll
                    for (int e = 0; e < 4; ++e) {
                        const auto sw2 = __builtin_amdgcn_permlane32_swap(__float_as_uint(acc[i][8 * j + e]),
                                                                          __float_as_uint(acc[i][8 * j + 4 + e]), false, false);
                        v[e] = __uint_as_float(sw2[0]);
                        v[4 + e] = __uint_as_float(sw2[1]);
                    }
                    v[0] += __uint_as_float(bq[j][0].x); v[1] += __uint_as_float(bq[j][0].y);
                    v[2] += __uint_as_float(bq[j][0].z); v[3] += __uint_as_float(bq[j][0].w);
                    v[4] += __uint_as_float(bq[j][1].x); v[5] += __uint_as_float(bq[j][1].y);
                    v[6] += __uint_as_float(bq[j][1].z); v[7] += __uint_as_float(bq[j][1].w);
                    alignas(16) E out[8];
                    Vec16<E>::store(out, v);
                    const uint4 ov = *reinterpret_cast<const uint4*>(out);
                    const unsigned yo = po < a.P && co < a.Cout ? ((unsigned)po * a.yLd + co) * 2u : FLAIR_OOB;
                    __builtin_amdgcn_raw_buffer_store_b128(u32x4_t{ov.x, ov.y, ov.z, ov.w}, yd, (int)yo, 0, 0);
                }
            }
            return;
        }
    }
#pragma unroll
    for (int i = 0; i < PAIRS; ++i) {
        const int pair = KSPLIT > 1 ? wave % NPAIR : wave * PAIRS + i;
        const int pfrag = pair % NPF, cf = pair / NPF;
        const long po = p0 + pfrag * 32 + lr;
        if (po >= a.P) continue;
#pragma unroll
        for (int g = 0; g < 4; ++g) {
            const int co = cf * 32 + 8 * g + 4 * lh;
            if (co >= a.Cout) continue;
            float v[4];
#pragma unroll
            for (int e = 0; e < 4; ++e) v[e] = acc[i][4 * g + e] + (a.bias ? a.bias[co + e] : 0.f);
            E* dst = y + po * a.yLd + co;
            if constexpr (sizeof(E) == 4) {
                *reinterpret_cast<float4*>(dst) = make_float4(v[0], v[1], v[2], v[3]);
            } else {
                uint2 pk;
                pk.x = pack2bf(v[0], v[1]);
                pk.y = pack2bf(v[2], v[3]);
                *reinterpret_cast<uint2*>(dst) = pk;
            }
        }
    }
}

}

template <typename E, int NCF, int NPF, int TPP, int OFFS, bool ONEFRAME, bool DOT2, int PFDSEL = 0>
static int launch_dcn_v2(const DcnArgs& a0, hipStream_t stream) {
    constexpr int PFD = PFDSEL > 0 ? PFDSEL : NCF >= 4 && TPP <= 8 ? 3 : 2;
    DcnArgs a = a0;
    if (ONEFRAME) {
        const unsigned long long half = a.Cin / 2, hw = (unsigned long long)a.H * a.W;
        a.xBytes[0] = (unsigned)(((hw - 1) * a.xLd[0] + half) * sizeof(E));
        a.xBytes[1] = (unsigned)(((hw - 1) * a.xLd[1] + half) * sizeof(E));
    }
    constexpr int NT = 32 * NPF * TPP, TP = 32 * NPF, TC = 32 * NCF;
    const int rawPitch = (OFFS == 2 ? (3 * a.G * (int)sizeof(E) + 15) & ~15 : 3 * a.G * (int)sizeof(E)) + 16;
    const size_t lds = (size_t)2 * TP * rawPitch + 2 * (TC + TP) * TPP * 16;
    static LdsAttrOnce attr;
    {
        const hipError_t e = flair_max_lds_once(attr, reinterpret_cast<const void*>(&dcn_kernel<E, NCF, NPF, TPP, OFFS, ONEFRAME, PFD, DOT2>));
        FLAIR_CHECK(e == hipSuccess, "flair_dcn_align: hipFuncSetAttribute: %s", hipGetErrorString(e));
    }
    hipLaunchKernelGGL((dcn_kernel<E, NCF, NPF, TPP, OFFS, ONEFRAME, PFD, DOT2>), dim3(cdiv(a.P, TP)), dim3(NT), lds, stream, a);
    FLAIR_LAUNCH_CHECK();
    return FLAIR_OK;
}

template <typename E, int NCF, int NPF, int TPP, int OFFS, bool ONEFRAME>
static int launch_dcn_v(const DcnArgs& a, hipStream_t stream) {
    if constexpr (sizeof(E) == 2 && OFFS == 1 && ONEFRAME) {
        if constexpr (NCF == 2 && NPF == 4) {
            return launch_dcn_v2<E, NCF, NPF, TPP, OFFS, ONEFRAME, true, 1>(a, stream);
        } else {
            return launch_dcn_v2<E, NCF, NPF, TPP, OFFS, ONEFRAME, true>(a, stream);
        }
    } else {
        return launch_dcn_v2<E, NCF, NPF, TPP, OFFS, ONEFRAME, false>(a, stream);
    }
}

template <typename E, int NCF, int NPF, int TPP>
static int launch_dcn(const DcnArgs& a, hipStream_t stream) {
    const bool oneframe = ((long)a.H * a.W) % (32 * NPF) == 0;
    if (a.activated && oneframe) return launch_dcn_v<E, NCF, NPF, TPP, 1, true>(a, stream);
    if (a.activated) return launch_dcn_v<E, NCF, NPF, TPP, 1, false>(a, stream);
    return launch_dcn_v<E, NCF, NPF, TPP, 0, false>(a, stream);
}

struct VqfrTile {
    int bke, tc;
};

static VqfrTile vqfr_tile(const flair_dcn_params* p) {
    if (p->dtype == FLAIR_BF16) {
        if ((p->Cin / 2) % 64 != 0) return {32, 64};
        if (p->Cout <= 64) return {64, 64};
        const long P = (long)p->F * p->H * p->W;
        return {P >= 64 * 256 && (p->Cin / 2) % 128 == 0 ? 128 : 64, 128};
    }
    return p->Cout <= 64 ? VqfrTile{16, 64} : VqfrTile{32, 128};
}

template <typename E>
static int launch_dcn_vqfr(const flair_dcn_params* p, const DcnArgs& a, hipStream_t stream) {
    if constexpr (sizeof(E) == 2) {
        if ((a.Cin / 2) % 64 != 0) return launch_dcn_v<E, 2, 4, 4, 2, false>(a, stream);
        if (a.Cout <= 64) return a.P >= 128 * 512 ? launch_dcn_v<E, 2, 4, 8, 2, false>(a, stream) : launch_dcn_v<E, 2, 2, 8, 2, false>(a, stream);
        if (a.P >= 64 * 256 && (a.Cin / 2) % 128 == 0) return launch_dcn_v<E, 4, 2, 16, 2, false>(a, stream);
        if (a.P >= 64 * 256) return launch_dcn_v<E, 4, 2, 8, 2, false>(a, stream);
        return launch_dcn_v<E, 4, 1, 8, 2, false>(a, stream);
    } else {
        (void)p;
        return a.Cout <= 64 ? launch_dcn_v<E, 2, 2, 4, 2, false>(a, stream) : launch_dcn_v<E, 4, 1, 8, 2, false>(a, stream);
    }
}

static int dcn_vqfr(const flair_dcn_params* p, const DcnArgs& a0, hipStream_t stream) {
    const VqfrTile t = vqfr_tile(p);
    const int esz = p->dtype == FLAIR_BF16 ? 2 : 4;
    for (int co0 = 0; co0 < p->Cout; co0 += t.tc) {
        DcnArgs a = a0;
        a.Cout = p->Cout - co0 < t.tc ? p->Cout - co0 : t.tc;
        a.w = static_cast<const char*>(a0.w) + (size_t)co0 * 9 * p->Cin * esz;
        a.bias = a0.bias ? a0.bias + co0 : nullptr;
        a.y = static_cast<char*>(a0.y) + (size_t)co0 * esz;
        a.wBytes = (unsigned)((unsigned long long)a.Cout * 9 * p->Cin * esz);
        const int rc = p->dtype == FLAIR_BF16 ? launch_dcn_vqfr<bf16_t>(p, a, stream) : launch_dcn_vqfr<float>(p, a, stream);
        if (rc != FLAIR_OK) return rc;
    }
    return FLAIR_OK;
}

extern "C" int flair_dcn_align(const flair_dcn_params* p, const void* x0, const void* x1, const void* raw,
                               const float* flow1, const float* flow2, const void* w, const float* bias, void* y,
                               hipStream_t stream) {
    FLAIR_CHECK(p && x0 && x1 && raw && w && y, "flair_dcn_align: null argument");
    FLAIR_CHECK(p->dtype == FLAIR_F32 || p->dtype == FLAIR_BF16, "flair_dcn_align: bad dtype");
    FLAIR_CHECK(p->raw_activated >= 0 && p->raw_activated <= 2, "flair_dcn_align: raw_activated = %d (0, 1 or 2)", p->raw_activated);
    const bool vqfr = p->raw_activated == 2;
    FLAIR_CHECK(!vqfr || (!flow1 && !flow2), "flair_dcn_align: raw_activated = 2 takes no flows");
    const int vec = p->dtype == FLAIR_BF16 ? 8 : 4;
    const int bke = vqfr ? vqfr_tile(p).bke : vec * (p->Cout <= 64 && p->dtype != FLAIR_BF16 ? 4 : 8);
    const int esz = p->dtype == FLAIR_BF16 ? 2 : 4;
    const int cpg = p->G > 0 ? p->Cin / p->G : 0;
    FLAIR_CHECK(p->G > 0 && (p->G % 8 == 0 || (vqfr && p->G == 4)) && p->G <= 16 && p->Cin % p->G == 0 && cpg % vec == 0 &&
                    (cpg & (cpg - 1)) == 0 && (p->Cin / 2) % bke == 0 && (!vqfr || p->Cin <= 1024),
                "flair_dcn_align: Cin=%d G=%d not supported", p->Cin, p->G);
    FLAIR_CHECK(p->Cout > 0 && p->Cout % 4 == 0 && (vqfr ? p->Cout <= 1024 : p->Cout <= 128) && p->raw_ld >= 27 * p->G &&
                    (p->raw_ld * esz) % 16 == 0,
                "flair_dcn_align: Cout = %d (a multiple of 4, <= 128; <= 1024 with raw_activated = 2) / raw_ld = %d (>= 27 G, "
                "16-byte granular)", p->Cout, p->raw_ld);
    FLAIR_CHECK(p->x_ld[0] >= p->Cin / 2 && p->x_ld[1] >= p->Cin / 2 && (p->x_ld[0] * esz) % 16 == 0 &&
                    (p->x_ld[1] * esz) % 16 == 0 && ((uintptr_t)x0) % 16 == 0 && ((uintptr_t)x1) % 16 == 0 &&
                    ((uintptr_t)raw) % 16 == 0 && p->y_ld >= p->Cout,
                "flair_dcn_align: strides/alignment (x_ld = %d, %d: >= Cin / 2 = %d, 16-byte granular; x0, x1, raw 16-byte "
                "aligned; y_ld = %d >= Cout = %d)", p->x_ld[0], p->x_ld[1], p->Cin / 2, p->y_ld, p->Cout);
    DcnArgs a;
    a.x[0] = x0; a.x[1] = x1; a.xLd[0] = p->x_ld[0]; a.xLd[1] = p->x_ld[1];
    a.Cin = p->Cin; a.raw = raw; a.rawLd = p->raw_ld; a.flow1 = flow1; a.flow2 = flow2;
    a.w = w; a.bias = bias; a.y = y; a.yLd = p->y_ld;
    a.F = p->F; a.H = p->H; a.W = p->W; a.Cout = p->Cout; a.G = p->G; a.maxMag = p->max_residue_magnitude;
    a.activated = p->raw_activated;
    a.P = (long)p->F * p->H * p->W;
    const unsigned long long half = p->Cin / 2;
    const unsigned long long b0 = ((unsigned long long)(a.P - 1) * p->x_ld[0] + half) * esz;
    const unsigned long long b1 = ((unsigned long long)(a.P - 1) * p->x_ld[1] + half) * esz;
    const unsigned long long br = ((unsigned long long)(a.P - 1) * p->raw_ld + 27 * p->G) * esz;
    const unsigned long long by = (unsigned long long)a.P * p->y_ld * esz;
    FLAIR_CHECK(b0 < 0x80000000ull && b1 < 0x80000000ull && br < 0x80000000ull && by < 0x80000000ull, "flair_dcn_align: tensor spans >= 2 GiB");
    FLAIR_CHECK(a.P + 2l * p->W + 2 < (1l << 23) && (long)p->x_ld[0] * esz < (1l << 23) && (long)p->x_ld[1] * esz < (1l << 23),
                "flair_dcn_align: F*H*W = %ld pixels (limit 2^23 per call: call per frame)", a.P);
    a.xBytes[0] = (unsigned)b0; a.xBytes[1] = (unsigned)b1; a.rawBytes = (unsigned)((br + 15) / 16 * 16);
    a.wBytes = (unsigned)((unsigned long long)p->Cout * 9 * p->Cin * esz);
    if (vqfr) return dcn_vqfr(p, a, stream);
    if (p->dtype == FLAIR_BF16) {
        if (p->Cout > 64) {
            if (a.P >= 64 * 256 && (p->Cin / 2) % 128 == 0) return launch_dcn<bf16_t, 4, 2, 16>(a, stream);
            if (a.P >= 64 * 256) return launch_dcn<bf16_t, 4, 2, 8>(a, stream);
            return launch_dcn<bf16_t, 4, 1, 8>(a, stream);
        }
        return a.P >= 128 * 512 ? launch_dcn<bf16_t, 2, 4, 8>(a, stream) : launch_dcn<bf16_t, 2, 2, 8>(a, stream);
    }
    return p->Cout <= 64 ? launch_dcn<float, 2, 2, 4>(a, stream) : launch_dcn<float, 4, 1, 8>(a, stream);
}
```

flair_amd/csrc/ew.hip:

```cpp
#include "common.h"

namespace {

template <typename E>
__global__ void nchw_to_nhwc_kernel(const float* src, int N, int C, long HW, E* dst, int ld, int coff) {
    const long total = (long)N * HW;
    for (long i = blockIdx.x * (long)blockDim.x + threadIdx.x; i < total; i += (long)gridDim.x * blockDim.x) {
        const long n = i / HW, p = i % HW;
        for (int c = 0; c < C; ++c) ET<E>::st(dst + i * ld + coff + c, src[(n * C + c) * HW + p]);
    }
}

template <typename E>
__global__ void nhwc_to_nchw_kernel(const E* src, int ld, int coff, int N, int C, long HW, float* dst) {
    const long total = (long)N * HW;
    for (long i = blockIdx.x * (long)blockDim.x + threadIdx.x; i < total; i += (long)gridDim.x * blockDim.x) {
        const long n = i / HW, p = i % HW;
        for (int c = 0; c < C; ++c) dst[(n * C + c) * HW + p] = ET<E>::ld(src + i * ld + coff + c);
    }
}

__global__ void timestep_embedding_kernel(const float* t, int N, int dim, float maxPeriod, int sinFirst,
                                          float* out) {
    const int half = dim / 2;
    const int i = blockIdx.x * blockDim.x + threadIdx.x;
    if (i >= N * half) return;
    const int n = i / half, k = i % half;
    const float freq = expf(-logf(maxPeriod) * (float)k / (float)half);
    const float arg = t[n] * freq;
    out[(long)n * dim + (sinFirst ? half : 0) + k] = cosf(arg);
    out[(long)n * dim + (sinFirst ? 0 : half) + k] = sinf(arg);
    if ((dim & 1) && k == 0) out[(long)n * dim + dim - 1] = 0.f;
}

template <int MMAX>
__global__ void linear_f32_kernel(const float* x, int M, int K, const float* w, const float* b, int N, int fpw,
                                  int actIn, int actOut, float* y, int yLd) {
    extern __shared__ float xs[];
    for (int i = threadIdx.x; i < M * K; i += blockDim.x) xs[i] = apply_act(x[i], actIn);
    __syncthreads();
    const int lane = threadIdx.x & 63;
    const int n0 = (blockIdx.x * (blockDim.x >> 6) + (threadIdx.x >> 6)) * fpw;
    for (int n = n0; n < n0 + fpw && n < N; ++n) {
        float acc[MMAX];
#pragma unroll
        for (int m = 0; m < MMAX; ++m) acc[m] = 0.f;
        const float* wr = w + (long)n * K;
        for (int k0 = lane; k0 < K; k0 += 64 * 8) {
            float wv[8];
#pragma unroll
            for (int j = 0; j < 8; ++j) wv[j] = k0 + 64 * j < K ? wr[k0 + 64 * j] : 0.f;
#pragma unroll
            for (int j = 0; j < 8; ++j) {
                const int k = k0 + 64 * j < K ? k0 + 64 * j : 0;
#pragma unroll
                for (int m = 0; m < MMAX; ++m)
                    if (m < M) acc[m] = fmaf(xs[m * K + k], wv[j], acc[m]);
            }
        }
#pragma unroll
        for (int m = 0; m < MMAX; ++m) {
            float v = acc[m];
#pragma unroll
            for (int off = 32; off > 0; off >>= 1) v += __shfl_xor(v, off);
            if (lane == 0 && m < M) y[(long)m * yLd + n] = apply_act(v + (b ? b[n] : 0.f), actOut);
        }
    }
}

__global__ void predict_xstart_kernel(const float* x, const float* modelOut, int N, int C, int Cm, long HW,
                                      float cRecip, float cRecipm1, int clip, float* x0) {
    const long total = (long)N * C * HW;
    for (long i = blockIdx.x * (long)blockDim.x + threadIdx.x; i < total; i += (long)gridDim.x * blockDim.x) {
        const long n = i / (C * HW), r = i % (C * HW);
        const float eps = modelOut[n * Cm * HW + r];
        float v = cRecip * x[i] - cRecipm1 * eps;
        if (clip) v = fminf(fmaxf(v, -1.f), 1.f);
        x0[i] = v;
    }
}

__global__ void sampler_update_kernel(const float* x, float* x0, const float* restored, const float* aux,
                                      const float* z, const float* prev, long frameElems, int T, int Tp,
                                      long total, float gamma, float wAux, float cRecip,
                                      float cRecipm1, float cPrev, float coNoise, float sq1mRho, float sqRho,
                                      int clip, int nonzero, float* xPrev) {
    for (long i = blockIdx.x * (long)blockDim.x + threadIdx.x; i < total; i += (long)gridDim.x * blockDim.x) {
        float v = x0[i];
        if (restored) {
            v = v - gamma * restored[i];
            if (clip) v = fminf(fmaxf(v, -1.f), 1.f);
        }
        if (aux) {
            float f = aux[i];
            if (clip) f = fminf(fmaxf(f, -1.f), 1.f);
            v = wAux * v + (1.f - wAux) * f;
        }
        if (prev) {
            const long n = i / frameElems, r = i % frameElems;
            const long b = n / T;
            const int t = (int)(n % T);
            if (t < Tp) v = prev[(b * Tp + t) * frameElems + r];
        }
        x0[i] = v;
        const float xi = x[i];
        const float eps = (cRecip * xi - v) / cRecipm1;
        float out = cPrev * v;
        if (nonzero) out += sq1mRho * coNoise * eps + sqRho * coNoise * z[i];
        xPrev[i] = out;
    }
}

__global__ void axpby_kernel(const float* x, const float* y, float a, float b, float lo, float hi, long n,
                             float* out) {
    for (long i = blockIdx.x * (long)blockDim.x + threadIdx.x; i < n; i += (long)gridDim.x * blockDim.x)
        out[i] = fminf(fmaxf(a * x[i] + (y ? b * y[i] : 0.f), lo), hi);
}

template <typename E>
__global__ void scale_pixels_kernel(E* x, int ld, int C, long P, const float* wmap) {
    constexpr int VEC = ET<E>::VEC;
    const int cv = C / VEC;
    const long total = P * cv;
    for (long i = blockIdx.x * (long)blockDim.x + threadIdx.x; i < total; i += (long)gridDim.x * blockDim.x) {
        const long p = i / cv;
        const int c0 = (int)(i % cv) * VEC;
        float v[VEC];
        Vec16<E>::load(x + p * ld + c0, v);
        const float s = wmap[p];
#pragma unroll
        for (int k = 0; k < VEC; ++k) v[k] *= s;
        Vec16<E>::store(x + p * ld + c0, v);
    }
}


__global__ void affine_channels_kernel(const float* x, int xLd, int C, long P, float a, float b, float lo,
                                       float hi, const float* sub, const float* mul, float* y, int yLd) {
    const long total = P * C;
    for (long i = blockIdx.x * (long)blockDim.x + threadIdx.x; i < total; i += (long)gridDim.x * blockDim.x) {
        const long p = i / C;
        const int c = (int)(i % C);
        float v = fminf(fmaxf(x[p * xLd + c] * a + b, lo), hi);
        y[p * yLd + c] = (v - (sub ? sub[c] : 0.f)) * (mul ? mul[c] : 1.f);
    }
}

template <typename E>
__global__ void add_frame_bias_kernel(E* x, int ld, int C, int F, long HW, const float* bias, int bLd) {
    const long total = (long)F * HW * C;
    for (long i = blockIdx.x * (long)blockDim.x + threadIdx.x; i < total; i += (long)gridDim.x * blockDim.x) {
        const int c = (int)(i % C);
// ... 66 lines not shown
        const int c0 = (int)(i % cv) * VEC;
        long q = i / cv;
        const int wo = (int)(q % Wo);
        q /= Wo;
        const int ho = (int)(q % Ho), f = (int)(q / Ho);
        float m[VEC];
#pragma unroll
        for (int k = 0; k < VEC; ++k) m[k] = -INFINITY;
        for (int dh = -1; dh <= 1; ++dh) {
            const int h = 2 * ho + dh;
            if ((unsigned)h >= (unsigned)H) continue;
            for (int dw = -1; dw <= 1; ++dw) {
                const int w = 2 * wo + dw;
                if ((unsigned)w >= (unsigned)W) continue;
                float v[VEC];
                Vec16<E>::load(x + (((long)f * H + h) * W + w) * xLd + c0, v);
#pragma unroll
                for (int k = 0; k < VEC; ++k) m[k] = fmaxf(m[k], v[k]);
            }
        }
        Vec16<E>::store(y + (((long)f * Ho + ho) * Wo + wo) * yLd + c0, m);
    }
}

inline int grid_for(long n, int block = 256, int cap = 2048) {
    long g = (n + block - 1) / block;
    if (g > cap) g = cap;
    if (g < 1) g = 1;
    return (int)g;
}

}

extern "C" int flair_nchw_f32_to_nhwc(const float* src, int N, int C, int H, int W, void* dst, int dtype,
                                      int dst_ld, int dst_coff, hipStream_t stream) {
    FLAIR_CHECK(src && dst && N > 0 && C > 0 && H > 0 && W > 0 && dst_coff >= 0 && dst_coff + C <= dst_ld,
                "flair_nchw_f32_to_nhwc: bad argument");
    const long HW = (long)H * W;
    if (dtype == FLAIR_BF16)
        hipLaunchKernelGGL(nchw_to_nhwc_kernel<bf16_t>, dim3(grid_for(N * HW)), dim3(256), 0, stream, src, N, C, HW,
                           (bf16_t*)dst, dst_ld, dst_coff);
    else if (dtype == FLAIR_F32)
        hipLaunchKernelGGL(nchw_to_nhwc_kernel<float>, dim3(grid_for(N * HW)), dim3(256), 0, stream, src, N, C, HW,
                           (float*)dst, dst_ld, dst_coff);
    else
        FLAIR_CHECK(false, "flair_nchw_f32_to_nhwc: bad dtype");
    FLAIR_LAUNCH_CHECK();
    return FLAIR_OK;
}

extern "C" int flair_nhwc_to_nchw_f32(const void* src, int dtype, int src_ld, int src_coff, int N, int C, int H,
                                      int W, float* dst, hipStream_t stream) {
    FLAIR_CHECK(src && dst && N > 0 && C > 0 && H > 0 && W > 0 && src_coff >= 0 && src_coff + C <= src_ld,
                "flair_nhwc_to_nchw_f32: bad argument");
    const long HW = (long)H * W;
    if (dtype == FLAIR_BF16)
        hipLaunchKernelGGL(nhwc_to_nchw_kernel<bf16_t>, dim3(grid_for(N * HW)), dim3(256), 0, stream,
                           (const bf16_t*)src, src_ld, src_coff, N, C, HW, dst);
    else if (dtype == FLAIR_F32)
        hipLaunchKernelGGL(nhwc_to_nchw_kernel<float>, dim3(grid_for(N * HW)), dim3(256), 0, stream,
                           (const float*)src, src_ld, src_coff, N, C, HW, dst);
    else
        FLAIR_CHECK(false, "flair_nhwc_to_nchw_f32: bad dtype");
    FLAIR_LAUNCH_CHECK();
    return FLAIR_OK;
}

extern "C" int flair_timestep_embedding(const float* t, int N, int dim, float max_period, int sin_first,
                                        float* out, hipStream_t stream) {
    FLAIR_CHECK(t && out && N > 0 && dim >= 2, "flair_timestep_embedding: bad argument");
    const int n = N * (dim / 2);
    hipLaunchKernelGGL(timestep_embedding_kernel, dim3((n + 255) / 256), dim3(256), 0, stream, t, N, dim, max_period,
                       sin_first, out);
    FLAIR_LAUNCH_CHECK();
    return FLAIR_OK;
}

extern "C" int flair_linear_f32(const float* x, int M, int K, const float* w, const float* bias, int N, int act_in,
                                int act_out, float* y, int y_ld, hipStream_t stream) {
    FLAIR_CHECK(x && w && y && M > 0 && M <= 32 && K > 0 && N > 0 && y_ld >= N, "flair_linear_f32: bad argument (M<=32)");
    const size_t lds = (size_t)M * K * sizeof(float);
    FLAIR_CHECK(lds <= 64 * 1024, "flair_linear_f32: M*K too large for LDS staging");
    const int wavesPerBlock = 4;
    const int fpw = N >= 8192 ? 8 : 1;
    const int grid = (N + wavesPerBlock * fpw - 1) / (wavesPerBlock * fpw);
    if (M <= 8)
        hipLaunchKernelGGL(linear_f32_kernel<8>, dim3(grid), dim3(256), lds, stream, x, M, K, w, bias, N, fpw,
                           act_in, act_out, y, y_ld);
    else if (M <= 16)
        hipLaunchKernelGGL(linear_f32_kernel<16>, dim3(grid), dim3(256), lds, stream, x, M, K, w, bias, N, fpw,
                           act_in, act_out, y, y_ld);
    else
        hipLaunchKernelGGL(linear_f32_kernel<32>, dim3(grid), dim3(256), lds, stream, x, M, K, w, bias, N, fpw,
                           act_in, act_out, y, y_ld);
    FLAIR_LAUNCH_CHECK();
    return FLAIR_OK;
}

extern "C" int flair_predict_xstart(const float* x, const float* model_out, int N, int C, int Cm, int H, int W,
                                    float c_recip, float c_recipm1, int clip, float* x0, hipStream_t stream) {
    FLAIR_CHECK(x && model_out && x0 && N > 0 && C > 0 && Cm >= C, "flair_predict_xstart: bad argument");
    const long HW = (long)H * W;
    hipLaunchKernelGGL(predict_xstart_kernel, dim3(grid_for((long)N * C * HW)), dim3(256), 0, stream, x, model_out, N,
                       C, Cm, HW, c_recip, c_recipm1, clip, x0);
    FLAIR_LAUNCH_CHECK();
    return FLAIR_OK;
}

extern "C" int flair_sampler_update(const flair_sampler_coefs* c, const float* x, float* x0, const float* restored,
                                    const float* aux, const float* z, const float* prev_recon, long n,
                                    float* x_prev, hipStream_t stream) {
    FLAIR_CHECK(c && x && x0 && x_prev && n > 0, "flair_sampler_update: null argument");
    FLAIR_CHECK(!c->nonzero || z, "flair_sampler_update: noise required when t != 0");
    FLAIR_CHECK(!prev_recon || (c->frame_elems > 0 && c->frames > 0 && c->prev_frames > 0 &&
                                c->prev_frames <= c->frames && n % (c->frame_elems * c->frames) == 0),
                "flair_sampler_update: prev_recon geometry");
    hipLaunchKernelGGL(sampler_update_kernel, dim3(grid_for(n)), dim3(256), 0, stream, x, x0, restored, aux, z,
                       prev_recon, (long)c->frame_elems, c->frames, c->prev_frames, n,
                       c->gamma, c->w_aux, c->sqrt_recip_alphas_cumprod, c->sqrt_recipm1_alphas_cumprod,
                       c->sqrt_alphas_cumprod_prev, c->sqrt_one_minus_alphas_cumprod_prev, c->sqrt_one_minus_rho,
                       c->sqrt_rho, c->clip_denoised, c->nonzero, x_prev);
    FLAIR_LAUNCH_CHECK();
    return FLAIR_OK;
}

extern "C" int flair_axpby_f32(const float* x, const float* y, float a, float b, float lo, float hi, long n,
                               float* out, hipStream_t stream) {
    FLAIR_CHECK(x && out && n > 0, "flair_axpby_f32: bad argument");
    hipLaunchKernelGGL(axpby_kernel, dim3(grid_for(n)), dim3(256), 0, stream, x, y, a, b, lo, hi, n, out);
    FLAIR_LAUNCH_CHECK();
    return FLAIR_OK;
}

extern "C" int flair_scale_pixels(void* x, int dtype, int ld, int C, long P, const float* wmap, hipStream_t stream) {
    FLAIR_CHECK(x && wmap && P > 0 && C > 0, "flair_scale_pixels: bad argument");
    FLAIR_CHECK(ld >= C && ld % (dtype == FLAIR_BF16 ? 8 : 4) == 0 && ((uintptr_t)x) % 16 == 0,
                "flair_scale_pixels: ld = %d (>= C = %d, 16-byte granular) / x alignment", ld, C);
    if (dtype == FLAIR_BF16) {
        FLAIR_CHECK(C % 8 == 0, "flair_scale_pixels: C %% 8");
        hipLaunchKernelGGL(scale_pixels_kernel<bf16_t>, dim3(grid_for(P * (C / 8))), dim3(256), 0, stream,
                           (bf16_t*)x, ld, C, P, wmap);
    } else {
        FLAIR_CHECK(C % 4 == 0, "flair_scale_pixels: C %% 4");
        hipLaunchKernelGGL(scale_pixels_kernel<float>, dim3(grid_for(P * (C / 4))), dim3(256), 0, stream, (float*)x,
                           ld, C, P, wmap);
    }
    FLAIR_LAUNCH_CHECK();
    return FLAIR_OK;
}

extern "C" int flair_affine_channels_f32(const float* x, int x_ld, int C, long P, float a, float b, float lo,
                                         float hi, const float* sub, const float* mul, float* y, int y_ld,
                                         hipStream_t stream) {
    FLAIR_CHECK(x && y && C > 0 && P > 0 && x_ld >= C && y_ld >= C, "flair_affine_channels_f32: bad argument");
    hipLaunchKernelGGL(affine_channels_kernel, dim3(grid_for(P * C)), dim3(256), 0, stream, x, x_ld, C, P, a, b, lo,
                       hi, sub, mul, y, y_ld);
    FLAIR_LAUNCH_CHECK();
    return FLAIR_OK;
}

extern "C" int flair_add_frame_bias(void* x, int dtype, int ld, int C, int F, long HW, const float* bias,
                                    int bias_ld, hipStream_t stream) {
    FLAIR_CHECK(x && bias && C > 0 && F > 0 && HW > 0 && ld >= C && bias_ld >= C, "flair_add_frame_bias: bad argument");
    if (dtype == FLAIR_BF16)
        hipLaunchKernelGGL(add_frame_bias_kernel<bf16_t>, dim3(grid_for(F * HW * C)), dim3(256), 0, stream,
                           (bf16_t*)x, ld, C, F, HW, bias, bias_ld);
// ... 109 lines not shown
```

flair_amd/guided_diffusion/unet_new.py:

```python
import math

import torch
import torch.nn as nn

from .. import ops
from .nn_new import conv_nd, linear, normalization, zero_module

A = ops


class PlaceHolder(nn.Module):

    def __init__(self, module):
        super().__init__()
        self.wrapped_module = module


LazyReshaper2D = LazyReshaper3D = PlaceHolder


class TemporalWrapper(PlaceHolder):
    """unet_new.py:50-59 (skipped when ``enable_cross_frames`` is False)."""


# ... 245 lines not shown
                    w2=_pack(rb.conv2.weight, [(c, c)], dtype, device), b2=_dev(rb.conv2.bias, device))




def run_trunk(pk, segs, c, *, extra_res=None, out=None, out_scale=1.0):
    k = (1, 3, 3)
    t1 = ops.conv(segs, pk["w0"], pk["b0"], c, k, act=A.ACT_LRELU01)
    if c == 64 and ops.chain_supported(t1, c):
        return ops.conv_chain(t1, pk["w1"], pk["b1"], A.ACT_RELU, pk["w2"], pk["b2"], A.ACT_NONE, c, c,
                              res0=t1, res1=extra_res, out=out, out_scale=out_scale)
    t2 = ops.conv(t1, pk["w1"], pk["b1"], c, k, act=A.ACT_RELU)
    return ops.conv(t2, pk["w2"], pk["b2"], c, k, res0=t1, res1=extra_res, out=out, out_scale=out_scale)


class SecondOrderDeformableAlignment(nn.Module):

    def __init__(self, in_channels, out_channels, kernel_size=3, padding=1, deform_groups=16,
                 max_residue_magnitude=10):
        super().__init__()
        assert kernel_size == 3 and padding == 1
        self.in_channels, self.out_channels = in_channels, out_channels
        self.deform_groups, self.max_residue_magnitude = deform_groups, max_residue_magnitude
        self.weight = nn.Parameter(torch.empty(out_channels, in_channels, 3, 3))
        self.bias = nn.Parameter(torch.zeros(out_channels))
        stdv = 1.0 / math.sqrt(in_channels * 9)
        with torch.no_grad():
            self.weight.uniform_(-stdv, stdv)
        c = out_channels
        self.conv_offset = nn.Sequential(
            nn.Conv2d(3 * c + 4, c, 3, 1, 1), nn.LeakyReLU(negative_slope=0.1),
            nn.Conv2d(c, c, 3, 1, 1), nn.LeakyReLU(negative_slope=0.1),
            nn.Conv2d(c, c, 3, 1, 1), nn.LeakyReLU(negative_slope=0.1),
            nn.Conv2d(c, 27 * deform_groups, 3, 1, 1))
        zero_module(self.conv_offset[-1])

    def pack(self, dtype, device):
        c = self.out_channels
        ka = ops.k_align(dtype)
        co = self.conv_offset
        perm = ops.dcn_raw_permutation(self.deform_groups)
        w6, b6 = co[6].weight.detach()[perm], co[6].bias.detach()[perm]
        return dict(
            w0=_pack(co[0].weight, [(c, c), (c, c), (c, c), (4, ka)], dtype, device), b0=_dev(co[0].bias, device),
            w2=_pack(co[2].weight, [(c, c)], dtype, device), b2=_dev(co[2].bias, device),
            w4=_pack(co[4].weight, [(c, c)], dtype, device), b4=_dev(co[4].bias, device),
            w6=_pack(w6, [(c, c)], dtype, device), b6=_dev(b6, device),
            wd=_pack(self.weight, [(2 * c, 2 * c)], dtype, device), bd=_dev(self.bias, device))


class BasicVSRPP(nn.Module):

    def __init__(self, mid_channels=64, max_residue_magnitude=10, use_checkpoint=False):
        super().__init__()
        self.mid_channels = mid_channels
        self.deform_align = nn.ModuleDict()
        self.backbone = nn.ModuleDict()
        for i, name in enumerate(["backward_1", "forward_1"]):
            self.deform_align[name] = SecondOrderDeformableAlignment(
                2 * mid_channels, mid_channels, 3, padding=1, deform_groups=16,
                max_residue_magnitude=max_residue_magnitude)
            self.backbone[name] = ResidualBlocksWithInputConv((2 + i) * mid_channels, mid_channels, 1)
        self.reconstruction = ResidualBlocksWithInputConv(3 * mid_channels, mid_channels, 1)
        self.conv_last = zero_module(nn.Conv2d(mid_channels, mid_channels, 1, 1))
        self._pk = None

    def pack(self, dtype, device):
        c = self.mid_channels
        self._pk = dict(
            align={n: m.pack(dtype, device) for n, m in self.deform_align.items()},
            trunk={"backward_1": self.backbone["backward_1"].pack(dtype, device, [c, c]),
                   "forward_1": self.backbone["forward_1"].pack(dtype, device, [c, c, c])},
            recon=self.reconstruction.pack(dtype, device, [c, c, c]),
            wl=_pack(self.conv_last.weight, [(c, c)], dtype, device), bl=_dev(self.conv_last.bias, device))

    def _propagate(self, ctx, hidden, flows, name, others, weight, wmaps, dest):
        pk_a, pk_t = self._pk["align"][name], self._pk["trunk"][name]
        T, H, W, c = hidden.shape
        order = list(range(T))
        flow_idx = list(range(-1, T - 1))
        if "backward" in name:
            order = order[::-1]
            flow_idx = order
        zero_c = torch.zeros((1, H, W, c), dtype=ctx.dtype, device=ctx.device)
        ka = ops.k_align(ctx.dtype)
        k3 = (1, 3, 3)
        G = self.deform_align[name].deform_groups
        mag = float(self.deform_align[name].max_residue_magnitude)
        store = ctx.flows.get("_prop") if isinstance(ctx.flows, dict) else None
        key = (name, H, W, ctx.dtype, ka)
        cached = store.get(key) if store is not None else None
        fill = [] if (cached is None and store is not None) else None
        prop, prev2 = zero_c, None
        for i, idx in enumerate(order):
            cur = hidden[idx:idx + 1]
            if i > 0:
                flow_n1 = flows[flow_idx[i]:flow_idx[i] + 1]
                cond_n1 = torch.empty_like(zero_c)
                second = i > 1
                feat_n2 = prev2 if second else zero_c
                cond_n2 = torch.empty_like(zero_c) if second else zero_c
                if cached is not None:
                    flow_n2, flowpad = cached[i - 1]
                    ops.vsrpp_warp2(prop, feat_n2 if second else None, flow_n1, flow_n2, cond_n1, cond_n2 if second else None)
                else:
                    flowpad = torch.zeros((1, H, W, ka), dtype=ctx.dtype, device=ctx.device)
                    flow_n2 = torch.empty_like(flow_n1) if second else None
                    ops.vsrpp_prep(prop, feat_n2 if second else None, flow_n1,
                                   flows[flow_idx[i - 1]:flow_idx[i - 1] + 1] if second else None,
                                   cond_n1, cond_n2 if second else None, flow_n2, flowpad)
                    if fill is not None:
                        fill.append((flow_n2, flowpad))
                o = ops.conv([cond_n1, cur, cond_n2, flowpad], pk_a["w0"], pk_a["b0"], c, k3, act=A.ACT_LRELU01)
                if c == 64 and ops.chain_supported(o, c):
                    o = ops.conv_chain(o, pk_a["w2"], pk_a["b2"], A.ACT_LRELU01, pk_a["w4"], pk_a["b4"],
                                       A.ACT_LRELU01, c, c)
                else:
                    o = ops.conv(o, pk_a["w2"], pk_a["b2"], c, k3, act=A.ACT_LRELU01)
                    o = ops.conv(o, pk_a["w4"], pk_a["b4"], c, k3, act=A.ACT_LRELU01)
                if c == 64 and ops.chain_supported(o, c) and W % 32 == 0:
                    raw = ops.conv_chain(o, None, None, A.ACT_NONE, pk_a["w6"], pk_a["b6"], A.ACT_DCN_OFFSETS, c, 27 * G,
                                         act_param=mag, act_period=3 * G)
                else:
                    raw = ops.conv(o, pk_a["w6"], pk_a["b6"], 27 * G, k3, act=A.ACT_DCN_OFFSETS, act_param=mag,
                                   act_period=3 * G)
                aligned = ops.dcn_align(prop, feat_n2, raw, flow_n1, flow_n2, pk_a["wd"], pk_a["bd"], c,
                                        groups=G, max_mag=mag, raw_activated=True)

            else:
                aligned = zero_c
            segs = [cur] + [o_[idx:idx + 1] for o_ in others] + [aligned]
            new = run_trunk(pk_t, segs, c, extra_res=aligned, out=dest[idx:idx + 1], out_scale=weight)
            if wmaps is not None:
                ops.scale_pixels(new, wmaps[idx])
            prev2, prop = (prop if i > 0 else None), new
        if fill is not None:
            store[key] = fill
        return dest

    def run(self, ctx, hidden):
        T, H, W, c = hidden.shape
        flows_forward, flows_backward = ctx.flows[W]
        weight, wmaps = 1.0, None
        vw = ctx.vsrpp_weights
        if isinstance(vw, (float, int)):
            weight = float(vw)
        elif vw is not None:
            wm = vw.reshape(T, vw.shape[-2], vw.shape[-1], 1).float().contiguous()
            if wm.shape[1] != H or wm.shape[2] != W:
                wm = ops.resize(wm, (H, W), ops.RESIZE_NEAREST)
            wmaps = [wm[i] for i in range(T)]
        bwd = torch.empty_like(hidden)
        fwd = torch.empty_like(hidden)
        self._propagate(ctx, hidden, flows_backward, "backward_1", [], weight, wmaps, bwd)
        ff = flows_forward if flows_forward is not None else flows_backward.flip(0)
        self._propagate(ctx, hidden, ff, "forward_1", [bwd], weight, wmaps, fwd)
        rec = run_trunk(self._pk["recon"], [hidden, bwd, fwd], c)
        return ops.conv(rec, self._pk["wl"], self._pk["bl"], c, (1, 1, 1), res0=hidden)


class _ConvModule(nn.Module):
    def __init__(self, cin, cout):
        super().__init__()
        self.conv = nn.Conv2d(cin, cout, kernel_size=7, stride=1, padding=3)


class SPyNetBasicModule(nn.Module):
    def __init__(self):
        super().__init__()
        ch = [8, 32, 64, 32, 16, 2]
        self.basic_module = nn.Sequential(*[_ConvModule(ch[i], ch[i + 1]) for i in range(5)])


class SPyNet(nn.Module):

    def __init__(self, pretrained=None):
        super().__init__()
        self.basic_module = nn.ModuleList([SPyNetBasicModule() for _ in range(6)])
        self.register_buffer("mean", torch.tensor([0.485, 0.456, 0.406]).view(1, 3, 1, 1))
        self.register_buffer("std", torch.tensor([0.229, 0.224, 0.225]).view(1, 3, 1, 1))
        self._pk = None

    def pack(self, device):
        f32 = torch.float32
        levels = []
        for bm in self.basic_module:
            convs = [m.conv for m in bm.basic_module]
            ws = [_pack(convs[0].weight, [(3, 4), (3, 4), (2, 8)], f32, device)]
            ws += [_pack(convs[j].weight, [(convs[j].in_channels,) * 2], f32, device) for j in (1, 2, 3)]
            ws.append(_pack(convs[4].weight, [(16, 16)], f32, device, cout_pad=4))
            bs = [_dev(convs[j].bias, device) for j in range(4)]
            bs.append(torch.cat([_dev(convs[4].bias, device), torch.zeros(2, device=device)]).contiguous())
            levels.append((ws, bs))
        mean = _dev(self.mean.reshape(-1), device)
        istd = (1.0 / _dev(self.std.reshape(-1), device)).contiguous()
        self._pk = dict(levels=levels, mean=mean, istd=istd)

    def run(self, ref, supp):
        F_, h0, w0, _ = ref.shape
        dev = ref.device
        if F_ == 0:
            return torch.zeros((0, h0, w0, 2), dtype=torch.float32, device=dev)
        h = h0 if h0 % 32 == 0 else 32 * (h0 // 32 + 1)
        w = w0 if w0 % 32 == 0 else 32 * (w0 // 32 + 1)
        if (h, w) != (h0, w0):
            ref = ops.resize(ref, (h, w), ops.RESIZE_BILINEAR, channels=3)
            supp = ops.resize(supp, (h, w), ops.RESIZE_BILINEAR, channels=3)
        sizes = [(h >> (5 - l), w >> (5 - l)) for l in range(6)]
        bufs = [torch.zeros((F_, *sizes[l], 16), dtype=torch.float32, device=dev) for l in range(6)]
        sp = [None] * 6
        ops.cast_channels(ref[..., :3], bufs[5], 0)
        sp[5] = supp
        for l in range(4, -1, -1):
# ... 322 lines not shown
```

flair_amd/ops.py:

```python
import ctypes

import torch

from . import _lib
from ._lib import (ACT_DCN_OFFSETS, ACT_GELU, ACT_LRELU01, ACT_LRELU02, ACT_NONE, ACT_RELU, ACT_SILU, ConvParams, check, dtype_code, lib,
                   ptr, stream)

__all__ = ["conv", "conv_chain", "group_norm", "nchw_to_clip", "clip_to_nchw", "timestep_embedding", "linear",
           "qkv_attention", "temporal_attention", "flow_warp", "flow_compose", "resize",
           "dcn_align", "dcn_raw_permutation", "scale_pixels", "predict_xstart", "sampler_update",
           "ACT_NONE", "ACT_RELU", "ACT_LRELU01", "ACT_SILU", "ACT_DCN_OFFSETS", "ACT_LRELU02", "ACT_GELU"]


class GnParams(ctypes.Structure):
    _fields_ = [("dtype", ctypes.c_int), ("C", ctypes.c_int), ("c0", ctypes.c_int),
                ("ld0", ctypes.c_int), ("ld1", ctypes.c_int), ("groups", ctypes.c_int),
                ("F", ctypes.c_int), ("H", ctypes.c_int), ("W", ctypes.c_int),
                ("frames_per_stat", ctypes.c_int), ("eps", ctypes.c_float), ("act", ctypes.c_int),
                ("resample", ctypes.c_int), ("y_ld", ctypes.c_int), ("raw_ld", ctypes.c_int),
                ("film_ld", ctypes.c_int)]


class SamplerCoefs(ctypes.Structure):
    _fields_ = [("gamma", ctypes.c_float), ("w_aux", ctypes.c_float),
                ("sqrt_recip_alphas_cumprod", ctypes.c_float),
                ("sqrt_recipm1_alphas_cumprod", ctypes.c_float),
                ("sqrt_alphas_cumprod_prev", ctypes.c_float),
                ("sqrt_one_minus_alphas_cumprod_prev", ctypes.c_float),
                ("sqrt_one_minus_rho", ctypes.c_float), ("sqrt_rho", ctypes.c_float),
                ("clip_denoised", ctypes.c_int), ("nonzero", ctypes.c_int),
                ("frame_elems", ctypes.c_long), ("frames", ctypes.c_int),
                ("prev_frames", ctypes.c_int)]


class AttnParams(ctypes.Structure):
    _fields_ = [("dtype", ctypes.c_int), ("frames", ctypes.c_int), ("L", ctypes.c_int),
                ("heads", ctypes.c_int), ("head_dim", ctypes.c_int), ("ld", ctypes.c_int),
                ("out_ld", ctypes.c_int), ("q_off", ctypes.c_int), ("k_off", ctypes.c_int),
                ("v_off", ctypes.c_int), ("head_stride", ctypes.c_int), ("scale", ctypes.c_float)]


class TAttnParams(ctypes.Structure):
    _fields_ = [("dtype", ctypes.c_int), ("T", ctypes.c_int), ("H", ctypes.c_int),
                ("W", ctypes.c_int), ("C", ctypes.c_int), ("window", ctypes.c_int),
                ("ld", ctypes.c_int), ("out_ld", ctypes.c_int), ("round_fp16", ctypes.c_int),
                ("scale", ctypes.c_float), ("head_dim", ctypes.c_int)]


class DcnParams(ctypes.Structure):
    _fields_ = [("dtype", ctypes.c_int), ("F", ctypes.c_int), ("H", ctypes.c_int),
                ("W", ctypes.c_int), ("Cin", ctypes.c_int), ("Cout", ctypes.c_int),
                ("G", ctypes.c_int), ("x_ld", ctypes.c_int * 2), ("raw_ld", ctypes.c_int),
                ("y_ld", ctypes.c_int), ("max_residue_magnitude", ctypes.c_float), ("raw_activated", ctypes.c_int)]


def _ld(t):
    assert t.dim() == 4 and t.stride(3) == 1, "clip tensors are (T,H,W,C) with C innermost"
    ld = t.stride(2)
    assert t.stride(1) == ld * t.shape[2] and (t.shape[0] == 1 or t.stride(0) == ld * t.shape[1] * t.shape[2]), \
        "clip tensor must be dense over (T,H,W)"
    return ld


def _f32(t):
    assert t is None or (t.dtype == torch.float32 and t.is_contiguous())
    return t


def k_align(dtype):
    return 32 if dtype == torch.bfloat16 else 16


def pad_channels(c, dtype):
    g = k_align(dtype)
    return (c + g - 1) // g * g


def conv(xs, weight, bias, cout, kernel, *, out=None, act=ACT_NONE, res0=None, res1=None,
         out_scale=1.0, stride=1, frame_bias=None, act_param=0.0, act_period=0, asym_pad=False, reflect_pad=False):
    if isinstance(xs, torch.Tensor):
        xs = [xs]
    x0 = xs[0]
    T, H, W, _ = x0.shape
    p = ConvParams()
    p.dtype = dtype_code(x0)
    p.T, p.H, p.W = T, H, W
    p.KT, p.KH, p.KW = kernel
    p.Cout = cout
    p.nseg = len(xs)
    arr = (ctypes.c_void_p * 4)()
    for i, x in enumerate(xs):
        assert x.dtype == x0.dtype and x.shape[:3] == x0.shape[:3]
        p.seg_c[i] = x.shape[3]
        p.seg_ld[i] = _ld(x)
        arr[i] = x.data_ptr()
    p.stride = stride
    p.asym_pad = int(asym_pad)
    p.reflect_pad = int(reflect_pad)
    p.frame_bias_ld = frame_bias.stride(0) if frame_bias is not None else 0
    if frame_bias is not None:
        assert frame_bias.dtype == torch.float32 and frame_bias.stride(1) == 1 and frame_bias.shape[0] == T
    Ho, Wo = (H + stride - 1) // stride, (W + stride - 1) // stride
    if out is None:
        out = torch.empty((T, Ho, Wo, cout), dtype=x0.dtype, device=x0.device)
    assert tuple(out.shape[:3]) == (T, Ho, Wo) and out.shape[3] >= cout and out.dtype == x0.dtype
    p.y_ld = _ld(out)
    p.res_ld[0] = _ld(res0) if res0 is not None else 0
    p.res_ld[1] = _ld(res1) if res1 is not None else 0
    p.act = act
    p.act_param, p.act_period = act_param, act_period
    p.out_scale = out_scale
    assert weight.dtype == x0.dtype and weight.is_contiguous()
    e0 = _prof_begin()
    wsb = _conv_ws_bytes(p)
    ws = _workspace(wsb, x0.device, "conv") if wsb else None

    def launch(_keep=xs):
        check(lib().flair_conv_nhwc(ctypes.byref(p), arr, ptr(weight), ptr(_f32(bias)), ptr(frame_bias), ptr(res0),
                                    ptr(res1), ptr(out), ptr(ws), ctypes.c_size_t(wsb), stream()), "flair_conv_nhwc")
    launch()
    if e0 is not None:
        cin = sum(x.shape[3] for x in xs)
        taps = kernel[0] * kernel[1] * kernel[2]
        esz = x0.element_size()
        flops = 2.0 * T * Ho * Wo * cout * cin * taps
        nbytes = esz * (cin * T * H * W + cout * T * Ho * Wo * (1 + (res0 is not None) + (res1 is not None))
                        + cout * taps * cin)
        _prof_end(e0, ("conv", lib().flair_conv_variant(ctypes.byref(p))), x0.dtype, flops, nbytes, launch,
                  ("conv", T, H, W, tuple(x.shape[3] for x in xs), cout, tuple(kernel), stride, act,
                   res0 is not None, res1 is not None, frame_bias is not None))
    return out


PROFILE = None


def _prof_begin():
    if PROFILE is None:
        return None
    e0 = torch.cuda.Event(enable_timing=True)
    e0.record()
    return e0


def _prof_end(e0, family, dtype, flops, nbytes, replay=None, sig=None):
    e1 = torch.cuda.Event(enable_timing=True)
    e1.record()
    PROFILE.append((family, str(dtype), float(flops), float(nbytes), e0, e1, replay, sig))


def conv_variant(T, H, W, cins, cout, kernel, dtype=torch.bfloat16, stride=1):
    p = ConvParams()
    p.dtype = 1 if dtype == torch.bfloat16 else 0
    p.T, p.H, p.W = T, H, W
    p.KT, p.KH, p.KW = kernel
    p.Cout = cout
    p.nseg = len(cins)
    for i, c in enumerate(cins):
        p.seg_c[i] = c
        p.seg_ld[i] = c
    p.stride = stride
    p.y_ld = cout
    return lib().flair_conv_variant(ctypes.byref(p))


def _conv_ws_bytes(p):
    f = lib().flair_conv_workspace_bytes
    f.restype = ctypes.c_size_t
    return f(ctypes.byref(p))


def pack_conv_weight(w, seg_channels, dtype, cout_pad=None):
    cout, cin = w.shape[:2]
    taps = 1
    for k in w.shape[2:]:
        taps *= k
    w = w.reshape(cout, cin, taps).permute(0, 2, 1).float()
    parts, o = [], 0
    for real, padded in seg_channels:
        seg = w[:, :, o:o + real]
        if padded > real:
            seg = torch.cat([seg, seg.new_zeros(cout, taps, padded - real)], dim=2)
        parts.append(seg)
        o += real
    assert o == cin, (o, cin)
    w = torch.cat(parts, dim=2)
    if cout_pad is not None and cout_pad > cout:
        w = torch.cat([w, w.new_zeros(cout_pad - cout, taps, w.shape[2])], dim=0)
    return w.to(dtype).contiguous()


class ChainParams(ctypes.Structure):
    _fields_ = [("dtype", ctypes.c_int), ("T", ctypes.c_int), ("H", ctypes.c_int), ("W", ctypes.c_int),
                ("C", ctypes.c_int), ("CoutB", ctypes.c_int), ("nseg", ctypes.c_int),
                ("seg_c", ctypes.c_int * 4), ("seg_ld", ctypes.c_int * 4), ("y_ld", ctypes.c_int),
                ("res_ld", ctypes.c_int * 2), ("actA", ctypes.c_int), ("actB", ctypes.c_int),
                ("out_scale", ctypes.c_float), ("act_param", ctypes.c_float), ("act_period", ctypes.c_int)]


def chain_supported(xs, c_mid):
    x0 = xs[0] if isinstance(xs, (list, tuple)) else xs
    T, H, W, _ = x0.shape
    tiles = T * ((H + 7) // 8) * (W // 32 if W % 32 == 0 and T * ((H + 7) // 8) * (W // 32) >= 192 else W // 8)
    return c_mid in (64, 128) and W % 8 == 0 and tiles <= 512


def conv_chain(xs, wA, bA, actA, wB, bB, actB, c_mid, coutB, *, res0=None, res1=None, out_scale=1.0, out=None,
               act_param=0.0, act_period=0):
    if isinstance(xs, torch.Tensor):
        xs = [xs]
    x0 = xs[0]
    T, H, W, _ = x0.shape
# ... 151 lines not shown
    p.scale = 1.0 / (d ** 0.5)
    e0 = _prof_begin()

    def launch():
        check(lib().flair_qkv_attention(ctypes.byref(p), ptr(qkv), ptr(out), stream()), "flair_qkv_attention")
    launch()
    if e0 is not None:
        L = H * W
        _prof_end(e0, ("attn", L), qkv.dtype, 4.0 * F_ * heads * L * L * d, qkv.element_size() * 4.0 * F_ * L * C,
                  launch, ("attn", F_, L, heads, d, new_order))
    return out


def temporal_attention(qkv, kpos, window, *, round_fp16, head_dim=64, out=None):
    T, H, W, C3 = qkv.shape
    C = C3 // 3
    p = TAttnParams()
    p.dtype = dtype_code(qkv)
    p.T, p.H, p.W, p.C, p.window = T, H, W, C, window
    p.ld = _ld(qkv)
    if out is None:
        out = torch.empty((T, H, W, C), dtype=qkv.dtype, device=qkv.device)
    p.out_ld = _ld(out)
    p.round_fp16 = int(round_fp16)
    p.head_dim = head_dim
    p.scale = 1.0 / (head_dim ** 0.5)
    assert kpos.shape == (window - 1, C)
    check(lib().flair_temporal_attention(ctypes.byref(p), ptr(qkv), ptr(_f32(kpos)), ptr(out), stream()),
          "flair_temporal_attention")
    return out


def flow_warp(x, flow, *, border=False, out=None):
    F_, H, W, C = x.shape
    assert flow.dtype == torch.float32 and flow.shape == (F_, H, W, 2)
    if out is None:
        out = torch.empty((F_, H, W, C), dtype=x.dtype, device=x.device)
    check(lib().flair_flow_warp(ptr(x), dtype_code(x), _ld(x), ptr(flow), _ld(flow), F_, H, W, C, int(border),
                                ptr(out), _ld(out), stream()), "flair_flow_warp")
    return out


def flow_compose(f1, f2, out=None):
    F_, H, W, _ = f1.shape
    assert f1.dtype == torch.float32 and f1.is_contiguous() and f2.is_contiguous()
    if out is None:
        out = torch.empty_like(f1)
    check(lib().flair_flow_compose(ptr(f1), ptr(f2), F_, H, W, ptr(out), stream()), "flair_flow_compose")
    return out


RESIZE_BILINEAR, RESIZE_BILINEAR_AC, RESIZE_BICUBIC, RESIZE_AVGPOOL2, RESIZE_NEAREST = 0, 1, 2, 3, 4


def resize(x, size, mode, *, channels=None, out=None, scale_c0=1.0, scale_c1=1.0):
    F_, Hi, Wi, Cx = x.shape
    C = channels or Cx
    Ho, Wo = size
    if out is None:
        out = torch.zeros((F_, Ho, Wo, Cx), dtype=x.dtype, device=x.device)
    check(lib().flair_resize_nhwc(ptr(x), dtype_code(x), _ld(x), F_, Hi, Wi, C, mode, Ho, Wo, ptr(out), _ld(out),
                                  ctypes.c_float(scale_c0), ctypes.c_float(scale_c1), stream()),
          "flair_resize_nhwc")
    return out


def dcn_raw_permutation(groups):
    G = groups
    perm = torch.empty(27 * G, dtype=torch.long)
    for k in range(9):
        for g in range(G):
            for e in range(2):
                perm[3 * G * k + 2 * g + e] = 2 * (g * 9 + k) + e
            perm[3 * G * k + 2 * G + g] = 18 * G + g * 9 + k
    return perm


def dcn_align(x0, x1, raw, flow1, flow2, weight, bias, cout, *, groups=16, max_mag=10.0, out=None, raw_activated=False):
    F_, H, W, ch = x0.shape
    p = DcnParams()
    p.dtype = dtype_code(x0)
    p.F, p.H, p.W = F_, H, W
    p.Cin, p.Cout, p.G = 2 * ch, cout, groups
    p.x_ld[0], p.x_ld[1] = _ld(x0), _ld(x1)
    p.raw_ld = _ld(raw)
    if out is None:
        out = torch.empty((F_, H, W, cout), dtype=x0.dtype, device=x0.device)
    p.y_ld = _ld(out)
    p.max_residue_magnitude = max_mag
    p.raw_activated = int(raw_activated)
    e0 = _prof_begin()

    def launch():
        check(lib().flair_dcn_align(ctypes.byref(p), ptr(x0), ptr(x1), ptr(raw), ptr(flow1), ptr(flow2), ptr(weight),
                                    ptr(_f32(bias)), ptr(out), stream()), "flair_dcn_align")
    launch()
    if e0 is not None:
        px = F_ * H * W
        _prof_end(e0, ("dcn", cout), x0.dtype, px * (2.0 * 9 * 2 * ch * cout + 9.0 * 2 * ch * 8),
                  x0.element_size() * px * (2 * ch + 27 * groups + cout), launch,
                  ("dcn", F_, H, W, ch, cout, groups, flow2 is not None))
    return out


def dcn_pack(x, raw, weight, bias, cout, *, groups, out=None):
    c = x.shape[3]
    assert c % 2 == 0
    return dcn_align(x[..., :c // 2], x[..., c // 2:], raw, None, None, weight, bias, cout, groups=groups, out=out,
                     raw_activated=2)


def scale_pixels(x, wmap):
    T, H, W, C = x.shape
    check(lib().flair_scale_pixels(ptr(x), dtype_code(x), _ld(x), C, ctypes.c_long(T * H * W), ptr(_f32(wmap)),
                                   stream()), "flair_scale_pixels")
    return x


def predict_xstart(x, model_out, c_recip, c_recipm1, clip, out=None):
    N, C, H, W = x.shape
    Cm = model_out.shape[1]
    assert x.dtype == torch.float32 and x.is_contiguous() and model_out.is_contiguous()
    if out is None:
        out = torch.empty_like(x)
    check(lib().flair_predict_xstart(ptr(x), ptr(model_out), N, C, Cm, H, W, ctypes.c_float(c_recip),
                                     ctypes.c_float(c_recipm1), int(clip), ptr(out), stream()),
          "flair_predict_xstart")
    return out


def sampler_update(coefs, x, x0, restored, aux, z, prev_recon, out=None):
    if out is None:
        out = torch.empty_like(x)
    for t in (x, x0, restored, aux, z, prev_recon):
        assert t is None or (t.dtype == torch.float32 and t.is_contiguous())
    check(lib().flair_sampler_update(ctypes.byref(coefs), ptr(x), ptr(x0), ptr(restored), ptr(aux), ptr(z),
                                     ptr(prev_recon), ctypes.c_long(x.numel()), ptr(out), stream()),
          "flair_sampler_update")
    return out


def affine_channels(x, C, a, b, lo, hi, sub, mul, out):
    T, H, W, _ = x.shape
    assert x.dtype == torch.float32 and out.dtype == torch.float32
    check(lib().flair_affine_channels_f32(ptr(x), _ld(x), C, ctypes.c_long(T * H * W), ctypes.c_float(a),
                                          ctypes.c_float(b), ctypes.c_float(lo), ctypes.c_float(hi), ptr(sub),
                                          ptr(mul), ptr(out), _ld(out), stream()), "flair_affine_channels_f32")
    return out


def add_frame_bias(x, bias):
    T, H, W, C = x.shape
    assert bias.dtype == torch.float32 and bias.stride(1) == 1
    check(lib().flair_add_frame_bias(ptr(x), dtype_code(x), _ld(x), C, T, ctypes.c_long(H * W), ptr(bias),
                                     bias.stride(0), stream()), "flair_add_frame_bias")
    return x


def cast_channels(src, dst, coff=0):
    T, H, W, C = src.shape
    assert src.dtype == torch.float32
    check(lib().flair_cast_channels(ptr(src), _ld(src), C, ctypes.c_long(T * H * W), ptr(dst), dtype_code(dst),
                                    _ld(dst), coff, stream()), "flair_cast_channels")
    return dst


def axpby(x, y, a, b, out=None, lo=float("-inf"), hi=float("inf")):
    assert x.dtype == torch.float32 and x.is_contiguous() and (y is None or y.is_contiguous())
    if out is None:
        out = torch.empty_like(x)
    check(lib().flair_axpby_f32(ptr(x), ptr(y), ctypes.c_float(a), ctypes.c_float(b), ctypes.c_float(lo),
                                ctypes.c_float(hi), ctypes.c_long(x.numel()), ptr(out), stream()),
          "flair_axpby_f32")
    return out


def learned_range_variance(model_out, C, min_log, max_log, out=None):
    N, C2, H, W = model_out.shape
    if out is None:
        var = torch.empty((N, C, H, W), dtype=torch.float32, device=model_out.device)
        logvar = torch.empty_like(var)
    else:
        var, logvar = out
# ... 317 lines not shown
```

Before: 0.8704.

## Skip all-zero conv/DCN input segments and add register-blocked small-M linear kernel

Conv and DCN kernels now accept absent (null) input segments, such as the zero tensors used for the first frame in propagation. They skip the matching K-range of channels and weights, indexing weights by a per-segment global offset (segW), and the split-K partitioning is recomputed over the present segments only. The Python propagation path passes None instead of zero tensors, so first-step convs do less MAC and load work. A separate register-held linear kernel for small M and K is also added. The change adds bookkeeping complexity in several kernels, and the DCN prologue now stages raw data during warm-up.

```diff
diff --git a/flair_amd/csrc/conv.hip b/flair_amd/csrc/conv.hip
--- a/flair_amd/csrc/conv.hip
+++ b/flair_amd/csrc/conv.hip
@@ -8,7 +8,9 @@
     const void* x[4];
     int segC[4];
     int segLd[4];
+    int segW[4];
     int nseg;
+    int CinRun;
     const void* w;
     const float* bias;
     const void* res0;
@@ -308,13 +310,12 @@
         ++cb;
         if (cb * BKE >= a.segC[seg]) {
             cb = 0;
-            segOff += a.segC[seg];
             if (++seg >= a.nseg) {
                 seg = 0;
-                segOff = 0;
                 ++dt;
                 while (dt <= pt && !dt_valid(dt)) ++dt;
             }
+            segOff = a.segW[seg];
         }
     };
     auto write_lds = [&](const uint4 (&hr)[HI], const uint4 (&wr)[WI]) {
@@ -332,7 +333,7 @@
     };
     int nValidDt = 0;
     for (int d = -pt; d <= pt; ++d) nValidDt += dt_valid(d) ? 1 : 0;
-    const int nch = nValidDt * (a.CinTot / BKE);
+    const int nch = nValidDt * (a.CinRun / BKE);
 
     f32x16 acc[RPW][2];
 #pragma unroll
@@ -583,13 +584,12 @@
         ++cb;
         if (cb * BKE >= a.segC[seg]) {
             cb = 0;
-            segOff += a.segC[seg];
             if (++seg >= a.nseg) {
                 seg = 0;
-                segOff = 0;
                 ++dt;
                 while (dt <= pt && !dt_valid(dt)) ++dt;
             }
+            segOff = a.segW[seg];
         }
     };
     auto write_lds = [&](int stage) {
@@ -609,7 +609,7 @@
     };
     int nValidDt = 0;
     for (int d = -pt; d <= pt; ++d) nValidDt += dt_valid(d) ? 1 : 0;
-    const int nch = nValidDt * (a.CinTot / BKE);
+    const int nch = nValidDt * (a.CinRun / BKE);
 
     f32x16 acc[RPW][CF];
 #pragma unroll
@@ -796,7 +796,7 @@
     const int wave = __builtin_amdgcn_readfirstlane(tid >> 6);
     const int lr = lane & 31, lh = lane >> 5;
     const int taps = a.KT * 9, pt = a.KT / 2;
-    const int chunksPerTap = a.CinTot / 32;
+    const int chunksPerTap = a.CinRun / 32;
     const int H = a.H, W = a.W, T = a.T;
 
     const int xcd = blockIdx.x & 7, slot = blockIdx.x >> 3, slotsPerXcd = gridDim.x >> 3;
@@ -861,14 +861,13 @@
         ++wk.cb;
         if (wk.cb * 32 >= a.segC[wk.seg]) {
             wk.cb = 0;
-            wk.segOff += a.segC[wk.seg];
             if (++wk.seg >= a.nseg) {
                 wk.seg = 0;
-                wk.segOff = 0;
                 ++wk.j;
                 while (wk.j < a.KT && (unsigned)(t + dt_at(t, wk.j)) >= (unsigned)T) ++wk.j;
                 wk.dt = dt_at(t, wk.j);
             }
+            wk.segOff = a.segW[wk.seg];
         }
     };
     auto chunks_of = [&](int t) {
@@ -1244,7 +1243,7 @@
     const int bid = xcd_remap(blockIdx.x, gridDim.x);
     const int t = bid / perFrame, tile = bid - t * perFrame;
     const int h0 = (tile / tilesW) * 8, w0 = (tile % tilesW) * 32;
-    const int nS = a.CinTot / 32;
+    const int nS = a.CinRun / 32;
 
     const u32x4_t wdesc = make_desc(a.w, a.wBytes);
     const u32x4_t bdesc = make_desc(a.bias, a.bias ? (unsigned)a.Cout * 4u : 0u);
@@ -1282,11 +1281,17 @@
             ++hseg;
         }
     };
+    int wseg = 0, wcb = 0;
     auto issue_w = [&](int s_) {
+        const unsigned kofs = (unsigned)(a.segW[wseg] + wcb * 32) * 2u;
 #pragma unroll
         for (int i = 0; i < NWS; ++i) {
             const int id = (wave * NWS + i) % WINSTR;
-            dma16(wdesc, wlane[i] == FLAIR_OOB ? FLAIR_OOB : wlane[i] + (unsigned)(s_ * 64), (unsigned)(RING + (s_ % WR) * SLOT + id * 1024));
+            dma16(wdesc, wlane[i] == FLAIR_OOB ? FLAIR_OOB : wlane[i] + kofs, (unsigned)(RING + (s_ % WR) * SLOT + id * 1024));
+        }
+        if (++wcb * 32 >= a.segC[wseg]) {
+            wcb = 0;
+            ++wseg;
         }
     };
     issue_halo(0);
@@ -1480,15 +1485,28 @@
 
     uint4 xreg[PD][XR], wreg[PD][WR];
 
-    const int nkAll = taps * (a.CinTot / BKE);
+    const int cpt = a.CinTot / BKE;
+    const int nkAll = taps * cpt;
     const int ks0 = (int)((long)blockIdx.y * nkAll / a.splitK);
     const int ks1 = (int)((long)(blockIdx.y + 1) * nkAll / a.splitK);
-    int tap = ks0 / (a.CinTot / BKE), seg = 0, cb = ks0 % (a.CinTot / BKE), segOff = 0;
-    while (cb * BKE >= a.segC[seg]) {
-        cb -= a.segC[seg] / BKE;
-        segOff += a.segC[seg];
-        ++seg;
-    }
+    int tap = 0, seg = 0, cb = 0, nk = taps * (a.CinRun / BKE);
+    if (a.splitK > 1) {
+        nk = 0;
+        bool found = false;
+        const int tap0 = ks0 / cpt, tap1 = (ks1 + cpt - 1) / cpt;
+        for (int tp = tap0; tp < tap1; ++tp)
+            for (int sg = 0; sg < a.nseg; ++sg) {
+                const int b = tp * cpt + a.segW[sg] / BKE, e = b + a.segC[sg] / BKE;
+                const int lo = b > ks0 ? b : ks0, hi = e < ks1 ? e : ks1;
+                if (hi <= lo) continue;
+                if (!found) {
+                    found = true;
+                    tap = tp; seg = sg; cb = lo - b;
+                }
+                nk += hi - lo;
+            }
+    }
+    int segOff = a.segW[seg];
     int dw = tap % a.KW - pw, dh = (tap / a.KW) % a.KH - ph, dt = tap / (a.KW * a.KH) - pt;
 
     const __amdgpu_buffer_rsrc_t wrs = make_rsrc(a.w, a.wBytes);
@@ -1527,11 +1545,9 @@
         ++cb;
         if (cb * BKE >= a.segC[seg]) {
             cb = 0;
-            segOff += a.segC[seg];
             ++seg;
             if (seg >= a.nseg) {
                 seg = 0;
-                segOff = 0;
                 ++tap;
                 ++dw;
                 if (dw > pw) {
@@ -1543,6 +1559,7 @@
                     }
                 }
             }
+            segOff = a.segW[seg];
         }
     };
     auto write_lds = [&](int buf, int set) {
@@ -1563,7 +1580,6 @@
 #pragma unroll
             for (int r = 0; r < 16; ++r) acc[i][j][r] = 0.f;
 
-    const int nk = ks1 - ks0;
     const int lr = lane & 31, lh = lane >> 5;
 
 #pragma unroll
@@ -1705,8 +1721,8 @@
 int launch(const ConvArgs& a, hipStream_t s) {
     if constexpr (sizeof(E) == 2) {
         bool ok = true;
-        for (int i = 0; i < a.nseg; ++i) ok = ok && a.segC[i] % 64 == 0;
-        if (ok) return launch_pd<E, TC, TP, WC, WP, 2, 2>(a, s);
+        for (int i = 0; i < a.nseg; ++i) ok = ok && a.segC[i] % 64 == 0 && a.segW[i] % 64 == 0;
+        if (ok && a.CinTot % 64 == 0) return launch_pd<E, TC, TP, WC, WP, 2, 2>(a, s);
     }
     return launch_pd<E, TC, TP, WC, WP, 4, 1>(a, s);
 }
@@ -1805,21 +1821,29 @@
     const int esz = p->dtype == FLAIR_BF16 ? 2 : 4;
     ConvArgs a{};
     a.CinTot = 0;
+    FLAIR_CHECK(x[0], "flair_conv_nhwc: segment 0 is null (only segments after the first may be absent)");
+    int n = 0;
     for (int i = 0; i < p->nseg; ++i) {
-        FLAIR_CHECK(x[i], "flair_conv_nhwc: segment %d is null", i);
         FLAIR_CHECK(p->seg_c[i] > 0 && p->seg_c[i] % bke == 0,
                     "flair_conv_nhwc: segment %d has %d channels; must be a multiple of %d", i, p->seg_c[i], bke);
+        if (!x[i]) {
+            a.CinTot += p->seg_c[i];
+            continue;
+        }
         FLAIR_CHECK(p->seg_ld[i] >= p->seg_c[i] && (p->seg_ld[i] * esz) % 16 == 0 &&
                         ((uintptr_t)x[i]) % 16 == 0,
                     "flair_conv_nhwc: segment %d stride/alignment", i);
-        a.x[i] = x[i];
-        a.segC[i] = p->seg_c[i];
-        a.segLd[i] = p->seg_ld[i];
+        a.x[n] = x[i];
+        a.segC[n] = p->seg_c[i];
+        a.segLd[n] = p->seg_ld[i];
+        a.segW[n] = a.CinTot;
+        a.CinRun += p->seg_c[i];
         a.CinTot += p->seg_c[i];
         const unsigned long long bytes = (unsigned long long)p->H * p->W * p->seg_ld[i] * esz;
         FLAIR_CHECK(bytes < 0x40000000ull, "flair_conv_nhwc: one frame of segment %d spans %llu bytes (limit 1 GiB)",
                     i, bytes);
-        a.segBytes[i] = (unsigned)bytes;
+        a.segBytes[n] = (unsigned)bytes;
+        ++n;
     }
     {
         const unsigned long long wb = (unsigned long long)p->Cout * p->KT * p->KH * p->KW * a.CinTot * esz;
@@ -1838,7 +1862,7 @@
                 p->res_ld[1], p->Cout, gran);
     FLAIR_CHECK(((uintptr_t)w) % 16 == 0, "flair_conv_nhwc: weight alignment");
     FLAIR_CHECK(!bias || ((uintptr_t)bias) % 16 == 0, "flair_conv_nhwc: bias alignment");
-    a.nseg = p->nseg;
+    a.nseg = n;
     a.w = w;
     a.bias = bias;
     a.fbias = frame_bias;
diff --git a/flair_amd/csrc/dcn.hip b/flair_amd/csrc/dcn.hip
--- a/flair_amd/csrc/dcn.hip
+++ b/flair_amd/csrc/dcn.hip
@@ -135,7 +135,7 @@
     int cpgShift = 0;
     while ((1 << cpgShift) < cpg) ++cpgShift;
     const int halfC = a.Cin / 2;
-    const int cbPerTap = a.Cin / BKE;
+    const int cbPerTap = (a.x[1] ? a.Cin : halfC) / BKE;
     const int nk = 9 * cbPerTap;
     const size_t fo0 = ONEFRAME ? (size_t)pf * a.H * a.W * a.xLd[0] * ESZ : 0, fo1 = ONEFRAME ? (size_t)pf * a.H * a.W * a.xLd[1] * ESZ : 0;
     const __amdgpu_buffer_rsrc_t xr0 = make_rsrc(reinterpret_cast<const char*>(a.x[0]) + fo0, a.xBytes[0]);
@@ -337,8 +337,15 @@
         }
     };
 #pragma unroll
-    for (int u = 0; u < PFD - 1; ++u)
+    for (int u = 0; u < PFD - 1; ++u) {
         if (u < nk) issue(rs[u]);
+        if (stageAt < 0 && stageTap < 9) {
+            __syncthreads();
+            stage_raw(stageTap);
+            ++stageTap;
+            stageAt += cbPerTap;
+        }
+    }
     constexpr int UNR = 2 * PFD;
     for (int k = 0; k < nk; k += UNR) {
 #pragma unroll
@@ -455,7 +462,7 @@
     if (ONEFRAME) {
         const unsigned long long half = a.Cin / 2, hw = (unsigned long long)a.H * a.W;
         a.xBytes[0] = (unsigned)(((hw - 1) * a.xLd[0] + half) * sizeof(E));
-        a.xBytes[1] = (unsigned)(((hw - 1) * a.xLd[1] + half) * sizeof(E));
+        a.xBytes[1] = a.x[1] ? (unsigned)(((hw - 1) * a.xLd[1] + half) * sizeof(E)) : 0u;
     }
     constexpr int NT = 32 * NPF * TPP, TP = 32 * NPF, TC = 32 * NCF;
     const int rawPitch = (OFFS == 2 ? (3 * a.G * (int)sizeof(E) + 15) & ~15 : 3 * a.G * (int)sizeof(E)) + 16;
@@ -538,11 +545,13 @@
 extern "C" int flair_dcn_align(const flair_dcn_params* p, const void* x0, const void* x1, const void* raw,
                                const float* flow1, const float* flow2, const void* w, const float* bias, void* y,
                                hipStream_t stream) {
-    FLAIR_CHECK(p && x0 && x1 && raw && w && y, "flair_dcn_align: null argument");
+    FLAIR_CHECK(p && x0 && raw && w && y, "flair_dcn_align: null argument");
     FLAIR_CHECK(p->dtype == FLAIR_F32 || p->dtype == FLAIR_BF16, "flair_dcn_align: bad dtype");
     FLAIR_CHECK(p->raw_activated >= 0 && p->raw_activated <= 2, "flair_dcn_align: raw_activated = %d (0, 1 or 2)", p->raw_activated);
     const bool vqfr = p->raw_activated == 2;
     FLAIR_CHECK(!vqfr || (!flow1 && !flow2), "flair_dcn_align: raw_activated = 2 takes no flows");
+    FLAIR_CHECK(x1 || !flow2, "flair_dcn_align: flow2 without x1 (a null x1 is an absent second half: flow2 must be null)");
+    FLAIR_CHECK(x1 || !vqfr, "flair_dcn_align: raw_activated = 2 needs both input halves (x1 is null)");
     const int vec = p->dtype == FLAIR_BF16 ? 8 : 4;
     const int bke = vqfr ? vqfr_tile(p).bke : vec * (p->Cout <= 64 && p->dtype != FLAIR_BF16 ? 4 : 8);
     const int esz = p->dtype == FLAIR_BF16 ? 2 : 4;
@@ -554,13 +563,13 @@
                     (p->raw_ld * esz) % 16 == 0,
                 "flair_dcn_align: Cout = %d (a multiple of 4, <= 128; <= 1024 with raw_activated = 2) / raw_ld = %d (>= 27 G, "
                 "16-byte granular)", p->Cout, p->raw_ld);
-    FLAIR_CHECK(p->x_ld[0] >= p->Cin / 2 && p->x_ld[1] >= p->Cin / 2 && (p->x_ld[0] * esz) % 16 == 0 &&
-                    (p->x_ld[1] * esz) % 16 == 0 && ((uintptr_t)x0) % 16 == 0 && ((uintptr_t)x1) % 16 == 0 &&
+    FLAIR_CHECK(p->x_ld[0] >= p->Cin / 2 && (!x1 || p->x_ld[1] >= p->Cin / 2) && (p->x_ld[0] * esz) % 16 == 0 &&
+                    (!x1 || (p->x_ld[1] * esz) % 16 == 0) && ((uintptr_t)x0) % 16 == 0 && ((uintptr_t)x1) % 16 == 0 &&
                     ((uintptr_t)raw) % 16 == 0 && p->y_ld >= p->Cout,
                 "flair_dcn_align: strides/alignment (x_ld = %d, %d: >= Cin / 2 = %d, 16-byte granular; x0, x1, raw 16-byte "
                 "aligned; y_ld = %d >= Cout = %d)", p->x_ld[0], p->x_ld[1], p->Cin / 2, p->y_ld, p->Cout);
     DcnArgs a;
-    a.x[0] = x0; a.x[1] = x1; a.xLd[0] = p->x_ld[0]; a.xLd[1] = p->x_ld[1];
+    a.x[0] = x0; a.x[1] = x1; a.xLd[0] = p->x_ld[0]; a.xLd[1] = x1 ? p->x_ld[1] : 0;
     a.Cin = p->Cin; a.raw = raw; a.rawLd = p->raw_ld; a.flow1 = flow1; a.flow2 = flow2;
     a.w = w; a.bias = bias; a.y = y; a.yLd = p->y_ld;
     a.F = p->F; a.H = p->H; a.W = p->W; a.Cout = p->Cout; a.G = p->G; a.maxMag = p->max_residue_magnitude;
@@ -568,11 +577,11 @@
     a.P = (long)p->F * p->H * p->W;
     const unsigned long long half = p->Cin / 2;
     const unsigned long long b0 = ((unsigned long long)(a.P - 1) * p->x_ld[0] + half) * esz;
-    const unsigned long long b1 = ((unsigned long long)(a.P - 1) * p->x_ld[1] + half) * esz;
+    const unsigned long long b1 = x1 ? ((unsigned long long)(a.P - 1) * p->x_ld[1] + half) * esz : 0;
     const unsigned long long br = ((unsigned long long)(a.P - 1) * p->raw_ld + 27 * p->G) * esz;
     const unsigned long long by = (unsigned long long)a.P * p->y_ld * esz;
     FLAIR_CHECK(b0 < 0x80000000ull && b1 < 0x80000000ull && br < 0x80000000ull && by < 0x80000000ull, "flair_dcn_align: tensor spans >= 2 GiB");
-    FLAIR_CHECK(a.P + 2l * p->W + 2 < (1l << 23) && (long)p->x_ld[0] * esz < (1l << 23) && (long)p->x_ld[1] * esz < (1l << 23),
+    FLAIR_CHECK(a.P + 2l * p->W + 2 < (1l << 23) && (long)p->x_ld[0] * esz < (1l << 23) && (long)a.xLd[1] * esz < (1l << 23),
                 "flair_dcn_align: F*H*W = %ld pixels (limit 2^23 per call: call per frame)", a.P);
     a.xBytes[0] = (unsigned)b0; a.xBytes[1] = (unsigned)b1; a.rawBytes = (unsigned)((br + 15) / 16 * 16);
     a.wBytes = (unsigned)((unsigned long long)p->Cout * 9 * p->Cin * esz);
diff --git a/flair_amd/csrc/ew.hip b/flair_amd/csrc/ew.hip
--- a/flair_amd/csrc/ew.hip
+++ b/flair_amd/csrc/ew.hip
@@ -68,6 +68,49 @@
     }
 }
 
+template <int MMAX>
+__global__ __launch_bounds__(256) void linear_f32_reg_kernel(const float* x, int M, int K, const float* w, const float* b, int N,
+                                                             int fpw, int actIn, int actOut, float* y, int yLd) {
+    static_assert(MMAX <= 16, "8 x MMAX input registers per lane");
+    extern __shared__ float xs[];
+    for (int i = threadIdx.x; i < M * K; i += blockDim.x) xs[i] = apply_act(x[i], actIn);
+    __syncthreads();
+    const int lane = threadIdx.x & 63;
+    float xr[8][MMAX];
+#pragma unroll
+    for (int j = 0; j < 8; ++j) {
+        const int k = lane + 64 * j < K ? lane + 64 * j : 0;
+#pragma unroll
+        for (int m = 0; m < MMAX; ++m) xr[j][m] = m < M ? xs[m * K + k] : 0.f;
+    }
+    const int n0 = (blockIdx.x * (blockDim.x >> 6) + (threadIdx.x >> 6)) * fpw;
+    const int n1 = n0 + fpw < N ? n0 + fpw : N;
+    float wv[8];
+#pragma unroll
+    for (int j = 0; j < 8; ++j) wv[j] = n0 < n1 && lane + 64 * j < K ? w[(long)n0 * K + lane + 64 * j] : 0.f;
+    for (int n = n0; n < n1; ++n) {
+        float wn[8];
+#pragma unroll
+        for (int j = 0; j < 8; ++j) wn[j] = n + 1 < n1 && lane + 64 * j < K ? w[(long)(n + 1) * K + lane + 64 * j] : 0.f;
+        float acc[MMAX];
+#pragma unroll
+        for (int m = 0; m < MMAX; ++m) acc[m] = 0.f;
+#pragma unroll
+        for (int j = 0; j < 8; ++j)
+#pragma unroll
+            for (int m = 0; m < MMAX; ++m) acc[m] = fmaf(xr[j][m], wv[j], acc[m]);
+#pragma unroll
+        for (int m = 0; m < MMAX; ++m) {
+            float v = acc[m];
+#pragma unroll
+            for (int off = 32; off > 0; off >>= 1) v += __shfl_xor(v, off);
+            if (lane == 0 && m < M) y[(long)m * yLd + n] = apply_act(v + (b ? b[n] : 0.f), actOut);
+        }
+#pragma unroll
+        for (int j = 0; j < 8; ++j) wv[j] = wn[j];
+    }
+}
+
 __global__ void predict_xstart_kernel(const float* x, const float* modelOut, int N, int C, int Cm, long HW,
                                       float cRecip, float cRecipm1, int clip, float* x0) {
     const long total = (long)N * C * HW;
@@ -300,6 +343,18 @@
     const size_t lds = (size_t)M * K * sizeof(float);
     FLAIR_CHECK(lds <= 64 * 1024, "flair_linear_f32: M*K too large for LDS staging");
     const int wavesPerBlock = 4;
+    if (M <= 16 && K <= 512) {
+        const int fpw = N >= 32768 ? 16 : N >= 8192 ? 8 : 1;
+        const int grid = (N + wavesPerBlock * fpw - 1) / (wavesPerBlock * fpw);
+        if (M <= 8)
+            hipLaunchKernelGGL(linear_f32_reg_kernel<8>, dim3(grid), dim3(256), lds, stream, x, M, K, w, bias, N, fpw,
+                               act_in, act_out, y, y_ld);
+        else
+            hipLaunchKernelGGL(linear_f32_reg_kernel<16>, dim3(grid), dim3(256), lds, stream, x, M, K, w, bias, N, fpw,
+                               act_in, act_out, y, y_ld);
+        FLAIR_LAUNCH_CHECK();
+        return FLAIR_OK;
+    }
     const int fpw = N >= 8192 ? 8 : 1;
     const int grid = (N + wavesPerBlock * fpw - 1) / (wavesPerBlock * fpw);
     if (M <= 8)
diff --git a/flair_amd/guided_diffusion/unet_new.py b/flair_amd/guided_diffusion/unet_new.py
--- a/flair_amd/guided_diffusion/unet_new.py
+++ b/flair_amd/guided_diffusion/unet_new.py
@@ -351,7 +351,6 @@
         if "backward" in name:
             order = order[::-1]
             flow_idx = order
-        zero_c = torch.zeros((1, H, W, c), dtype=ctx.dtype, device=ctx.device)
         ka = ops.k_align(ctx.dtype)
         k3 = (1, 3, 3)
         G = self.deform_align[name].deform_groups
@@ -360,24 +359,24 @@
         key = (name, H, W, ctx.dtype, ka)
         cached = store.get(key) if store is not None else None
         fill = [] if (cached is None and store is not None) else None
-        prop, prev2 = zero_c, None
+        prop, prev2 = None, None
         for i, idx in enumerate(order):
             cur = hidden[idx:idx + 1]
             if i > 0:
                 flow_n1 = flows[flow_idx[i]:flow_idx[i] + 1]
-                cond_n1 = torch.empty_like(zero_c)
+                cond_n1 = torch.empty_like(cur)
                 second = i > 1
-                feat_n2 = prev2 if second else zero_c
-                cond_n2 = torch.empty_like(zero_c) if second else zero_c
+                feat_n2 = prev2 if second else None
+                cond_n2 = torch.empty_like(cur) if second else None
                 if cached is not None:
                     flow_n2, flowpad = cached[i - 1]
-                    ops.vsrpp_warp2(prop, feat_n2 if second else None, flow_n1, flow_n2, cond_n1, cond_n2 if second else None)
+                    ops.vsrpp_warp2(prop, feat_n2, flow_n1, flow_n2, cond_n1, cond_n2)
                 else:
                     flowpad = torch.zeros((1, H, W, ka), dtype=ctx.dtype, device=ctx.device)
                     flow_n2 = torch.empty_like(flow_n1) if second else None
-                    ops.vsrpp_prep(prop, feat_n2 if second else None, flow_n1,
+                    ops.vsrpp_prep(prop, feat_n2, flow_n1,
                                    flows[flow_idx[i - 1]:flow_idx[i - 1] + 1] if second else None,
-                                   cond_n1, cond_n2 if second else None, flow_n2, flowpad)
+                                   cond_n1, cond_n2, flow_n2, flowpad)
                     if fill is not None:
                         fill.append((flow_n2, flowpad))
                 o = ops.conv([cond_n1, cur, cond_n2, flowpad], pk_a["w0"], pk_a["b0"], c, k3, act=A.ACT_LRELU01)
@@ -397,7 +396,7 @@
                                         groups=G, max_mag=mag, raw_activated=True)
 
             else:
-                aligned = zero_c
+                aligned = None
             segs = [cur] + [o_[idx:idx + 1] for o_ in others] + [aligned]
             new = run_trunk(pk_t, segs, c, extra_res=aligned, out=dest[idx:idx + 1], out_scale=weight)
             if wmaps is not None:
diff --git a/flair_amd/ops.py b/flair_amd/ops.py
--- a/flair_amd/ops.py
+++ b/flair_amd/ops.py
@@ -82,6 +82,10 @@
         xs = [xs]
     x0 = xs[0]
     T, H, W, _ = x0.shape
+    if any(x is None for x in xs):
+        assert sum(x is None for x in xs) == 1, "one None segment (its width is inferred); give the others as int widths"
+        rest = weight.shape[-1] - sum(x if isinstance(x, int) else x.shape[3] for x in xs if x is not None)
+        xs = [rest if x is None else x for x in xs]
     p = ConvParams()
     p.dtype = dtype_code(x0)
     p.T, p.H, p.W = T, H, W
@@ -90,6 +94,9 @@
     p.nseg = len(xs)
     arr = (ctypes.c_void_p * 4)()
     for i, x in enumerate(xs):
+        if isinstance(x, int):
+            p.seg_c[i] = x
+            continue
         assert x.dtype == x0.dtype and x.shape[:3] == x0.shape[:3]
         p.seg_c[i] = x.shape[3]
         p.seg_ld[i] = _ld(x)
@@ -120,14 +127,15 @@
                                     ptr(res1), ptr(out), ptr(ws), ctypes.c_size_t(wsb), stream()), "flair_conv_nhwc")
     launch()
     if e0 is not None:
-        cin = sum(x.shape[3] for x in xs)
+        present = [x for x in xs if not isinstance(x, int)]
+        cin = sum(x.shape[3] for x in present)
         taps = kernel[0] * kernel[1] * kernel[2]
         esz = x0.element_size()
         flops = 2.0 * T * Ho * Wo * cout * cin * taps
         nbytes = esz * (cin * T * H * W + cout * T * Ho * Wo * (1 + (res0 is not None) + (res1 is not None))
                         + cout * taps * cin)
         _prof_end(e0, ("conv", lib().flair_conv_variant(ctypes.byref(p))), x0.dtype, flops, nbytes, launch,
-                  ("conv", T, H, W, tuple(x.shape[3] for x in xs), cout, tuple(kernel), stride, act,
+                  ("conv", T, H, W, tuple(x.shape[3] for x in present), cout, tuple(kernel), stride, act,
                    res0 is not None, res1 is not None, frame_bias is not None))
     return out
 
@@ -445,7 +453,7 @@
     p.dtype = dtype_code(x0)
     p.F, p.H, p.W = F_, H, W
     p.Cin, p.Cout, p.G = 2 * ch, cout, groups
-    p.x_ld[0], p.x_ld[1] = _ld(x0), _ld(x1)
+    p.x_ld[0], p.x_ld[1] = _ld(x0), (_ld(x1) if x1 is not None else 0)
     p.raw_ld = _ld(raw)
     if out is None:
         out = torch.empty((F_, H, W, cout), dtype=x0.dtype, device=x0.device)
@@ -460,8 +468,9 @@
     launch()
     if e0 is not None:
         px = F_ * H * W
-        _prof_end(e0, ("dcn", cout), x0.dtype, px * (2.0 * 9 * 2 * ch * cout + 9.0 * 2 * ch * 8),
-                  x0.element_size() * px * (2 * ch + 27 * groups + cout), launch,
+        cw = 2 * ch if x1 is not None else ch
+        _prof_end(e0, ("dcn", cout), x0.dtype, px * (2.0 * 9 * cw * cout + 9.0 * cw * 8),
+                  x0.element_size() * px * (cw + 27 * groups + cout), launch,
                   ("dcn", F_, H, W, ch, cout, groups, flow2 is not None))
     return out
 
```

New measurement: 0.8709 (median of 3 runs). No clear change (+0.1%).
